# naturerobots/mesh_navigation

Measured on AMD Instinct MI355X. Metric: plans/sec (Dijkstra makePlan device path incl. computeVectorMap, 1M-vertex mesh), higher is better.
Workload: dtype f32

## Files before the change

### include/mnav.h

```cpp
#ifndef MNAV_H
#define MNAV_H

#include <stdint.h>

#ifdef __cplusplus
extern "C" {
#endif

#define MNAV_SUCCESS 0u
#define MNAV_CANCELED 51u
#define MNAV_INVALID_START 52u
#define MNAV_INVALID_GOAL 53u
#define MNAV_NO_PATH_FOUND 54u
#define MNAV_INTERNAL_ERROR 60u
#define MNAV_NONE 0xFFFFFFFFu

typedef struct mnav_ctx mnav_ctx;

typedef struct mnav_stats {
  uint32_t steps;
  uint32_t launches;
  uint32_t bands;
  uint32_t armed;
  float goal_dist;
// ... 73 lines not shown
                        const float* sensor_to_map, const float* down_axis, double robot_height, double max_obstacle_dist,
                        uint32_t* changed_out, uint32_t* n_changed, uint32_t* n_lethal);
int mnav_obstacle_stats(const mnav_ctx* ctx, uint32_t* rays_kept, uint32_t* hits, uint32_t* lethal_rays, float* ms_bvh_build,
                        float* ms_cast, float* ms_total);
int mnav_layer_height_diff(mnav_ctx* ctx, uint32_t layer, double radius, double threshold);
int mnav_layer_roughness(mnav_ctx* ctx, uint32_t layer, double radius, double threshold);
int mnav_layer_ridge(mnav_ctx* ctx, uint32_t layer, double radius, double threshold);
int mnav_neighbourhood_stats(const mnav_ctx* ctx, uint32_t* centres, uint64_t* visits, uint32_t* max_size,
                             uint32_t* spilled, float* ms);
int mnav_layer_border(mnav_ctx* ctx, uint32_t layer, double border_cost, double threshold, uint32_t* changed_out, uint32_t* n_changed,
                      uint32_t* n_lethal);
int mnav_layer_clearance(mnav_ctx* ctx, uint32_t layer, double robot_height, double height_inflation, uint32_t* changed_out,
                         uint32_t* n_changed, uint32_t* n_lethal);
int mnav_clearance_download(const mnav_ctx* ctx, float* clearance_out);
int mnav_clearance_stats(const mnav_ctx* ctx, uint32_t* cast, uint32_t* rays, uint32_t* hits, float* ms_bvh_build, float* ms_cast,
                         float* ms_total);

enum { MNAV_NODE_INPUT = 0, MNAV_NODE_INFLATION = 1, MNAV_NODE_COMBINE_MAX = 2, MNAV_NODE_COMBINE_AVG = 3 };
typedef struct {
  uint32_t layer;
  uint32_t kind;
  uint32_t n_inputs;
  uint32_t inputs[8];
  float    weights[8];
  double   inflation_radius, inscribed_radius, inscribed_value, lethal_value, cost_scaling_factor;
} mnav_map_node;
int mnav_map_configure(mnav_ctx* ctx, uint32_t n_nodes, const mnav_map_node* nodes, uint32_t default_layer, double edge_cost_factor,
                       const uint8_t* invalid);
int mnav_map_compute(mnav_ctx* ctx);
int mnav_map_layer_changed(mnav_ctx* ctx, uint32_t layer, uint32_t n, const uint32_t* vertex_ids, uint32_t* changed_out, uint32_t* n_changed);
int mnav_map_update_layer(mnav_ctx* ctx, uint32_t layer, uint32_t n, const uint32_t* vertex_ids, const float* costs, const uint8_t* lethal,
                          uint32_t* changed_out, uint32_t* n_changed);
int mnav_map_obstacle(mnav_ctx* ctx, uint32_t layer, uint32_t n_points, const void* points, uint32_t point_step, const float* sensor_to_map,
                      const float* down_axis, double robot_height, double max_obstacle_dist, uint32_t* changed_out, uint32_t* n_changed);
int mnav_map_stats(const mnav_ctx* ctx, uint32_t* waves, uint32_t* recombined, uint32_t* default_changed, uint32_t* edges_reweighted,
                   float* ms_total, float* ms_wave);

uint32_t mnav_replan_dijkstra_batch(mnav_ctx* ctx, uint32_t n, const uint32_t* targets, double goal_dist_offset, uint32_t* codes_out,
                                    float* dist_out, uint32_t* pred_out, uint32_t* path_out, uint32_t path_cap, uint32_t* path_len);
uint32_t mnav_replan_plans(const mnav_ctx* ctx);
int mnav_replan_stats(const mnav_ctx* ctx, uint32_t* reason, uint32_t* log_len, float* levels_out, uint64_t* kept, uint64_t* rewound,
                      uint32_t* tiles_woken, uint32_t* rounds, float* ms_level, float* ms_rewind, float* ms_rounds, float* ms_finalize);

uint32_t mnav_replan_dijkstra_each(mnav_ctx* ctx, uint32_t n, const uint32_t* targets, double goal_dist_offset, uint32_t* codes_out,
                                   float* dist_out, uint32_t* pred_out, uint32_t* path_out, uint32_t path_cap, uint32_t* path_len);
int mnav_replan_each_stats(const mnav_ctx* ctx, uint32_t* reason, uint32_t* whole_fresh, uint32_t* log_len, uint8_t* classes_out,
                           float* levels_out, uint32_t* counts, uint64_t* kept, uint64_t* rewound, uint32_t* tiles_woken, uint32_t* rounds,
                           int32_t* fresh_engine, float* ms);

int mnav_replan_warm_stats(const mnav_ctx* ctx, uint32_t* plans, uint32_t* kernel, uint32_t* iterations, uint64_t* pairs_woken, uint64_t* words,
                           float* ms, uint32_t* fallback, uint32_t* live);

int mnav_locate(mnav_ctx* ctx, uint32_t n, const float* pos, uint32_t* vertex_out, uint32_t* face_out, float* bary_out,
                float* dist_out);
int mnav_locate_stats(const mnav_ctx* ctx, uint32_t* built, float* ms_build, float* ms_query, uint64_t* candidates);
uint32_t mnav_plan_dijkstra_batch_at(mnav_ctx* ctx, uint32_t n, const float* goal_pos, const float* start_pos,
                                     double goal_dist_offset, double cost_limit, uint32_t* codes_out, uint32_t* seeds_out,
                                     uint32_t* targets_out, float* dist_out, uint32_t* pred_out, uint32_t* path_out,
                                     uint32_t path_cap, uint32_t* path_len);
uint32_t mnav_plan_cvp_batch_at(mnav_ctx* ctx, uint32_t n, const float* goal_pos, const float* start_pos,
                                double goal_dist_offset, double cost_limit, uint32_t* codes_out, uint32_t* seed_faces_out,
                                uint32_t* target_faces_out, float* dist_out, uint32_t* pred_out, float* vecmap_out);

typedef struct mnav_follow_config {
  double max_lin_velocity;
  double max_ang_velocity;
  double arrival_fading;
  double ang_vel_factor;
  double lin_vel_factor;
  double max_angle;
  double max_search_radius;
  double max_search_distance;
} mnav_follow_config;
#define MNAV_FOLLOW_CONFIG_DEFAULTS { 1.0, 0.5, 0.5, 1.0, 1.0, 20.0, 0.4, 0.4 }
enum { MNAV_FOLLOW_OK = 0, MNAV_FOLLOW_OUT_OF_MAP = 1, MNAV_FOLLOW_NO_FIELD = 2 };
int mnav_follow_batch(mnav_ctx* ctx, uint32_t n, const float* pos, const float* dir, const float* up, const uint32_t* face_in,
                      const uint32_t* slots, const uint32_t* seed_faces, const mnav_follow_config* config, int32_t* code_out,
                      uint32_t* face_out, float* bary_out, float* pos_out, float* mesh_dir_out, float* cost_out, double* cmd_out,
                      int32_t* how_out);
int mnav_follow_stats(const mnav_ctx* ctx, uint32_t* stayed, uint32_t* neighbour, uint32_t* global, uint32_t* lost,
                      uint32_t* no_field, uint32_t* built_index, float* ms_kernels, float* ms_total);

enum { MNAV_ROLLOUT_RUNNING = 0, MNAV_ROLLOUT_REACHED = 1, MNAV_ROLLOUT_OUT_OF_MAP = 2, MNAV_ROLLOUT_NO_FIELD = 3 };
typedef struct mnav_rollout_config {
  double   dt;
  double   dist_tolerance;
  double   angle_tolerance;
  uint32_t ticks;
  uint32_t trace_stride;
} mnav_rollout_config;
int mnav_follow_rollout(mnav_ctx* ctx, uint32_t n, const float* pos, const float* dir, const float* up, const uint32_t* face_in,
                        const uint32_t* slots, const uint32_t* seed_faces, const float* goal_pos, const float* goal_dir,
                        const mnav_follow_config* config, const mnav_rollout_config* rollout, int32_t* status_out,
                        uint32_t* ticks_out, float* pos_out, float* dir_out, uint32_t* face_out, double* travel_out,
                        double* cost_integral_out, float* min_goal_dist_out, float* trace_out);
int mnav_rollout_stats(const mnav_ctx* ctx, uint32_t* status_counts, uint64_t* robot_ticks, uint64_t* stayed, uint64_t* neighbour,
                       uint64_t* global, uint32_t* built_index, float* ms_kernels, float* ms_total);

#define MNAV_BEYOND_FIELD 70u
int mnav_fleet_paths(mnav_ctx* ctx, uint32_t n, const uint32_t* slots, const uint32_t* start_vertex, const float* start_pos,
                     uint32_t* code_out, uint32_t* vertex_out, float* potential_out, uint32_t* len_out, uint64_t* offset_out,
                     uint32_t* ids_out, uint64_t ids_cap, uint64_t* total_out);
int mnav_fleet_walks(mnav_ctx* ctx, uint32_t n, const uint32_t* slots, uint32_t n_plans, const float* seed_pos,
                     const uint32_t* seed_faces, const float* start_pos, const uint32_t* start_faces, double step_width,
                     int32_t inflation_layer, uint32_t walk_cap, int32_t* status_out, uint32_t* start_face_out, uint32_t* len_out,
                     uint64_t* offset_out, float* positions_out, uint32_t* faces_out, uint64_t entries_cap, uint64_t* total_out);
int mnav_upload_face_normals(mnav_ctx* ctx, uint32_t F, const float* face_normals);
int mnav_fleet_plans(mnav_ctx* ctx, uint32_t n, const uint32_t* slots, const uint32_t* start_vertex, const float* start_pos,
                     uint32_t n_plans, const float* goal_pos, uint32_t* code_out, uint32_t* vertex_out, float* potential_out,
                     uint32_t* len_out, uint64_t* offset_out, double* cost_out, double* poses_out, uint64_t poses_cap,
                     uint64_t* total_out);
int mnav_fleet_walk_plans(mnav_ctx* ctx, uint32_t n, const uint32_t* slots, uint32_t n_plans, const float* seed_pos,
                          const uint32_t* seed_faces, const double* goal_pose, const float* start_pos, const uint32_t* start_faces,
                          double step_width, int32_t inflation_layer, uint32_t walk_cap, int32_t* status_out,
                          uint32_t* start_face_out, uint32_t* len_out, uint64_t* offset_out, double* cost_out, double* poses_out,
                          uint64_t poses_cap, uint64_t* total_out);
int mnav_fleet_stats(const mnav_ctx* ctx, uint32_t* served, uint32_t* beyond_field, uint32_t* no_path, uint32_t* invalid,
                     uint64_t* entries, uint32_t* built_index, uint32_t* chunks, float* ms_kernels, float* ms_total);

int mnav_shard_setup(mnav_ctx* ctx, uint32_t rank, uint32_t world);
int mnav_shard_info(const mnav_ctx* ctx, uint32_t* t_lo, uint32_t* t_hi, uint32_t* ntiles, uint32_t* n_exchange);
int mnav_shard_setup_partition(mnav_ctx* ctx, uint32_t n_exchange, const uint32_t* exchange_vertex, const uint8_t* owned);
int mnav_shard_walk(mnav_ctx* ctx, uint32_t start_vertex, uint32_t seed_vertex, uint32_t cap, uint32_t* out_host);
uint64_t mnav_device_bytes(const mnav_ctx* ctx);

int mnav_shard_begin(mnav_ctx* ctx, uint32_t seed_vertex, uint32_t target_vertex, double goal_dist_offset, double cost_limit);
int mnav_shard_set_goal_tie(mnav_ctx* ctx, uint32_t tie_id);
int mnav_shard_rounds(mnav_ctx* ctx, uint32_t rounds, float* iface_buf_dev);
int mnav_shard_apply(mnav_ctx* ctx, const float* iface_buf_dev, float* local_min_out, float* target_dist_out);
int mnav_shard_finalize(mnav_ctx* ctx, float* dist_buf_dev, uint32_t* pred_buf_dev);
int mnav_shard_rounds_async(mnav_ctx* ctx, uint32_t rounds, float* iface_buf_dev, void* caller_stream);
int mnav_shard_apply_async(mnav_ctx* ctx, const float* iface_buf_dev, float* ctl_dev, void* caller_stream);

void mnav_cancel(mnav_ctx* ctx);

int mnav_get_stats(const mnav_ctx* ctx, mnav_stats* out);
int mnav_get_timing(const mnav_ctx* ctx, mnav_stats* out);
int mnav_set_band_width(mnav_ctx* ctx, float delta);
int mnav_set_dijkstra_engine(mnav_ctx* ctx, int engine);
int mnav_set_option(mnav_ctx* ctx, const char* name, double value);
double mnav_get_option(const mnav_ctx* ctx, const char* name);
int mnav_set_resident_outputs(mnav_ctx* ctx, int on);
int mnav_download_output(mnav_ctx* ctx, uint32_t slot, int what, void* host_out);
int mnav_vector_at(mnav_ctx* ctx, uint32_t slot, const uint32_t vs[3], const float bary[3], float out[3]);
int mnav_backtrack_cvp_batch(mnav_ctx* ctx, uint32_t n, const float* seed_pos, const uint32_t* seed_faces, const float* target_pos,
                             const uint32_t* target_faces, double step_width, int32_t inflation_layer, uint32_t cap,
                             float* positions_out, uint32_t* faces_out, uint32_t* n_out, int32_t* status_out);
int mnav_backtrack_cvp(mnav_ctx* ctx, const float seed_pos[3], uint32_t seed_face, const float target_pos[3], uint32_t target_face,
                       double step_width, int32_t inflation_layer, uint32_t cap, float* positions_out, uint32_t* faces_out,
                       uint32_t* n_out);
const void* mnav_device_output(const mnav_ctx* ctx, uint32_t slot, int what);
uint64_t mnav_algorithmic_bytes(const mnav_ctx* ctx);
int mnav_last_engine(const mnav_ctx* ctx);

#ifdef __cplusplus
}
#endif
#endif
```

### mesh_navigation_amd/capi.py

```python
from __future__ import annotations

import ctypes as C
import os
import sys
import time
import weakref
from dataclasses import dataclass

import numpy as np

from . import build as _build

NONE = 0xFFFFFFFF
SUCCESS, CANCELED, INVALID_START, INVALID_GOAL, NO_PATH_FOUND, INTERNAL_ERROR = 0, 51, 52, 53, 54, 60
BEYOND_FIELD = 70
WALK_NO_FACE = -3

SYMBOLS = [
    "mnav_create", "mnav_destroy", "mnav_last_error", "mnav_set_face_circulation", "mnav_upload_mesh", "mnav_upload_costs",
    "mnav_compute_edge_weights", "mnav_combine_costs", "mnav_plan_dijkstra", "mnav_plan_cvp", "mnav_plan_dijkstra_batch", "mnav_plan_cvp_batch",
    "mnav_cancel", "mnav_get_stats", "mnav_get_timing", "mnav_set_band_width", "mnav_set_dijkstra_engine", "mnav_device_output",
    "mnav_algorithmic_bytes", "mnav_shard_setup", "mnav_shard_setup_partition", "mnav_shard_walk", "mnav_device_bytes", "mnav_shard_info", "mnav_shard_begin", "mnav_shard_rounds", "mnav_shard_apply", "mnav_shard_rounds_async", "mnav_shard_apply_async",
    "mnav_shard_finalize", "mnav_update_costs", "mnav_update_edge_weights", "mnav_download_costs", "mnav_set_resident_outputs", "mnav_download_output",
    "mnav_vector_at", "mnav_backtrack_cvp", "mnav_backtrack_cvp_batch", "mnav_layer_upload", "mnav_layer_steepness", "mnav_layer_inflation", "mnav_layer_download",
    "mnav_combine_layers", "mnav_layer_stats", "mnav_layer_download_vectors", "mnav_combine_layers_update",
    "mnav_layer_obstacle", "mnav_obstacle_stats",
    "mnav_layer_height_diff", "mnav_layer_roughness", "mnav_layer_ridge", "mnav_neighbourhood_stats",
    "mnav_layer_border", "mnav_layer_clearance", "mnav_clearance_download", "mnav_clearance_stats",
    "mnav_locate", "mnav_locate_stats", "mnav_plan_dijkstra_batch_at", "mnav_plan_cvp_batch_at",
    "mnav_follow_batch", "mnav_follow_stats", "mnav_follow_rollout", "mnav_rollout_stats",
    "mnav_map_configure", "mnav_map_compute", "mnav_map_layer_changed", "mnav_map_update_layer", "mnav_map_obstacle", "mnav_map_stats",
    "mnav_replan_dijkstra_batch", "mnav_replan_plans", "mnav_replan_stats", "mnav_replan_dijkstra_each", "mnav_replan_each_stats",
    "mnav_replan_warm_stats",
    "mnav_fleet_paths", "mnav_fleet_walks", "mnav_fleet_stats",
    "mnav_upload_face_normals", "mnav_fleet_plans", "mnav_fleet_walk_plans",
    "mnav_set_option", "mnav_get_option", "mnav_shard_set_goal_tie", "mnav_last_engine",
]


class _PathRows:

    def __init__(self, buf, lens, cap):
        self._buf, self._lens, self._cap = buf, lens, cap

    def __len__(self):
        return self._lens.shape[0]

    def __getitem__(self, k):
        if isinstance(k, slice):
            return [self[i] for i in range(*k.indices(len(self)))]
        if k < 0:
            k += len(self)
        return self._buf[k, : min(int(self._lens[k]), self._cap)].copy()

    def __iter__(self):
        return (self[i] for i in range(len(self)))


class Stats(C.Structure):
    _fields_ = [("steps", C.c_uint32), ("launches", C.c_uint32), ("bands", C.c_uint32), ("armed", C.c_uint32),
                ("goal_dist", C.c_float), ("n_plans", C.c_uint32), ("evals", C.c_uint64), ("settled", C.c_uint64),
                ("ms_init", C.c_float), ("ms_propagation", C.c_float), ("ms_vector_map", C.c_float),
                ("ms_path", C.c_float), ("ms_download", C.c_float), ("ms_total", C.c_float), ("ms_step_kernels", C.c_float),
                ("band_shrinks", C.c_uint32), ("band_cuts", C.c_uint32)]

    def as_dict(self) -> dict:
        return {k: getattr(self, k) for k, _ in self._fields_}


class FollowConfig(C.Structure):
    _fields_ = [("max_lin_velocity", C.c_double), ("max_ang_velocity", C.c_double), ("arrival_fading", C.c_double),
                ("ang_vel_factor", C.c_double), ("lin_vel_factor", C.c_double), ("max_angle", C.c_double),
                ("max_search_radius", C.c_double), ("max_search_distance", C.c_double)]
    DEFAULTS = dict(max_lin_velocity=1.0, max_ang_velocity=0.5, arrival_fading=0.5, ang_vel_factor=1.0, lin_vel_factor=1.0,
                    max_angle=20.0, max_search_radius=0.4, max_search_distance=0.4)

    def __init__(self, **kw):
        super().__init__(**{**self.DEFAULTS, **kw})


FOLLOW_OK, FOLLOW_OUT_OF_MAP, FOLLOW_NO_FIELD = 0, 1, 2


class RolloutConfig(C.Structure):
    _fields_ = [("dt", C.c_double), ("dist_tolerance", C.c_double), ("angle_tolerance", C.c_double), ("ticks", C.c_uint32),
                ("trace_stride", C.c_uint32)]
    DEFAULTS = dict(dt=0.1, dist_tolerance=0.2, angle_tolerance=0.8, ticks=1, trace_stride=0)

    def __init__(self, **kw):
        super().__init__(**{**self.DEFAULTS, **kw})


ROLLOUT_RUNNING, ROLLOUT_REACHED, ROLLOUT_OUT_OF_MAP, ROLLOUT_NO_FIELD = 0, 1, 2, 3


class MapNode(C.Structure):
    _fields_ = [("layer", C.c_uint32), ("kind", C.c_uint32), ("n_inputs", C.c_uint32), ("inputs", C.c_uint32 * 8),
                ("weights", C.c_float * 8), ("inflation_radius", C.c_double), ("inscribed_radius", C.c_double),
                ("inscribed_value", C.c_double), ("lethal_value", C.c_double), ("cost_scaling_factor", C.c_double)]


NODE_KINDS = {"input": 0, "inflation": 1, "max": 2, "avg": 3}


@dataclass
class FollowOut:
    code: np.ndarray | None
    face: np.ndarray | None
    bary: np.ndarray | None
    pos: np.ndarray | None
    mesh_dir: np.ndarray | None
    cost: np.ndarray | None
    cmd: np.ndarray | None
    how: np.ndarray | None


@dataclass
class RolloutOut:
    status: np.ndarray | None
    ticks: np.ndarray | None
    pos: np.ndarray | None
    dir: np.ndarray | None
    face: np.ndarray | None
    travel: np.ndarray | None
    cost_integral: np.ndarray | None
    min_goal_dist: np.ndarray | None
    trace: np.ndarray | None
    cancelled: bool = False


_lib = None


def load(path: str | None = None):
    global _lib
    if _lib is not None and path is None:
        return _lib
    p = path or os.environ.get("MNAV_LIB") or _build.LIB
    if path is None and not os.path.exists(p):
        _build.build_lib()
    if not os.path.exists(p):
        raise RuntimeError(f"HIP library {p} is missing -- run `python -m mesh_navigation_amd.build`")
    L = C.CDLL(p)
    vp, u32, f64 = C.c_void_p, C.c_uint32, C.c_double
    L.mnav_create.restype = vp
    L.mnav_create.argtypes = [C.c_int]
    L.mnav_destroy.argtypes = [vp]
    L.mnav_last_error.restype = C.c_char_p
    L.mnav_last_error.argtypes = [vp]
    L.mnav_set_face_circulation.restype = C.c_int
    L.mnav_set_face_circulation.argtypes = [vp, u32, u32, vp, vp]
    L.mnav_upload_mesh.restype = C.c_int
    L.mnav_upload_mesh.argtypes = [vp, u32, u32, u32, vp, vp, vp, vp]
    L.mnav_upload_costs.restype = C.c_int
    L.mnav_upload_costs.argtypes = [vp, vp, vp, vp]
    L.mnav_compute_edge_weights.restype = C.c_int
    L.mnav_compute_edge_weights.argtypes = [vp, vp, vp, f64, vp, vp]
    L.mnav_combine_costs.restype = C.c_int
    L.mnav_combine_costs.argtypes = [vp, C.c_int, u32, vp, vp, vp, f64, vp, vp, vp]
    L.mnav_plan_dijkstra.restype = u32
    L.mnav_plan_dijkstra.argtypes = [vp, u32, u32, f64, f64, vp, vp, vp, u32, C.POINTER(u32), vp]
    L.mnav_plan_cvp.restype = u32
    L.mnav_plan_cvp.argtypes = [vp, vp, u32, u32, f64, f64, vp, vp, vp, vp, vp]
    L.mnav_plan_dijkstra_batch.restype = u32
    L.mnav_plan_dijkstra_batch.argtypes = [vp, u32, vp, vp, f64, f64, vp, vp, vp, vp, u32, vp]
    L.mnav_plan_cvp_batch.restype = u32
    L.mnav_plan_cvp_batch.argtypes = [vp, u32, vp, vp, vp, f64, f64, vp, vp, vp, vp]
    L.mnav_locate.restype = C.c_int
    L.mnav_locate.argtypes = [vp, u32, vp, vp, vp, vp, vp]
    L.mnav_locate_stats.restype = C.c_int
    L.mnav_locate_stats.argtypes = [vp, C.POINTER(u32), C.POINTER(C.c_float), C.POINTER(C.c_float), C.POINTER(C.c_uint64)]
    L.mnav_plan_dijkstra_batch_at.restype = u32
    L.mnav_plan_dijkstra_batch_at.argtypes = [vp, u32, vp, vp, f64, f64, vp, vp, vp, vp, vp, vp, u32, vp]
    L.mnav_plan_cvp_batch_at.restype = u32
    L.mnav_plan_cvp_batch_at.argtypes = [vp, u32, vp, vp, f64, f64, vp, vp, vp, vp, vp, vp]
    L.mnav_follow_batch.restype = C.c_int
    L.mnav_follow_batch.argtypes = [vp, u32, vp, vp, vp, vp, vp, vp, C.POINTER(FollowConfig), vp, vp, vp, vp, vp, vp, vp, vp]
    L.mnav_follow_stats.restype = C.c_int
    L.mnav_follow_stats.argtypes = [vp] + [C.POINTER(u32)] * 6 + [C.POINTER(C.c_float)] * 2
    L.mnav_follow_rollout.restype = C.c_int
    L.mnav_follow_rollout.argtypes = [vp, u32] + [vp] * 8 + [C.POINTER(FollowConfig), C.POINTER(RolloutConfig)] + [vp] * 9
    L.mnav_rollout_stats.restype = C.c_int
    L.mnav_rollout_stats.argtypes = [vp, C.POINTER(u32 * 4)] + [C.POINTER(C.c_uint64)] * 4 + [C.POINTER(u32)] + [C.POINTER(C.c_float)] * 2
    L.mnav_map_configure.restype = C.c_int
    L.mnav_map_configure.argtypes = [vp, u32, C.POINTER(MapNode), u32, f64, vp]
    L.mnav_map_compute.restype = C.c_int
    L.mnav_map_compute.argtypes = [vp]
    L.mnav_map_layer_changed.restype = C.c_int
    L.mnav_map_layer_changed.argtypes = [vp, u32, u32, vp, vp, C.POINTER(u32)]
    L.mnav_map_update_layer.restype = C.c_int
    L.mnav_map_update_layer.argtypes = [vp, u32, u32, vp, vp, vp, vp, C.POINTER(u32)]
    L.mnav_map_obstacle.restype = C.c_int
    L.mnav_map_obstacle.argtypes = [vp, u32, u32, vp, u32, vp, vp, f64, f64, vp, C.POINTER(u32)]
    L.mnav_map_stats.restype = C.c_int
    L.mnav_map_stats.argtypes = [vp] + [C.POINTER(u32)] * 4 + [C.POINTER(C.c_float)] * 2
    L.mnav_replan_dijkstra_batch.restype = u32
    L.mnav_replan_dijkstra_batch.argtypes = [vp, u32, vp, f64, vp, vp, vp, vp, u32, vp]
    L.mnav_replan_dijkstra_each.restype = u32
    L.mnav_replan_dijkstra_each.argtypes = [vp, u32, vp, f64, vp, vp, vp, vp, u32, vp]
    L.mnav_replan_each_stats.restype = C.c_int
    L.mnav_replan_each_stats.argtypes = ([vp] + [C.POINTER(u32)] * 3 + [vp, vp, vp] + [C.POINTER(C.c_uint64)] * 2 + [C.POINTER(u32)] * 2
                                         + [C.POINTER(C.c_int32), vp])
    L.mnav_replan_warm_stats.restype = C.c_int
    L.mnav_replan_warm_stats.argtypes = [vp] + [C.POINTER(u32)] * 3 + [C.POINTER(C.c_uint64)] * 2 + [vp] + [C.POINTER(u32)] * 2
    L.mnav_replan_plans.restype = u32
    L.mnav_replan_plans.argtypes = [vp]
    L.mnav_replan_stats.restype = C.c_int
    L.mnav_replan_stats.argtypes = [vp, C.POINTER(u32), C.POINTER(u32), vp] + [C.POINTER(C.c_uint64)] * 2 + [C.POINTER(u32)] * 2 + [C.POINTER(C.c_float)] * 4
    L.mnav_cancel.argtypes = [vp]
    L.mnav_get_stats.restype = C.c_int
    L.mnav_get_stats.argtypes = [vp, C.POINTER(Stats)]
    L.mnav_get_timing.restype = C.c_int
    L.mnav_get_timing.argtypes = [vp, C.POINTER(Stats)]
    L.mnav_set_band_width.restype = C.c_int
    L.mnav_set_band_width.argtypes = [vp, C.c_float]
    L.mnav_set_dijkstra_engine.restype = C.c_int
    L.mnav_set_dijkstra_engine.argtypes = [vp, C.c_int]
    L.mnav_shard_set_goal_tie.restype = C.c_int
    L.mnav_shard_set_goal_tie.argtypes = [vp, u32]
    L.mnav_set_option.restype = C.c_int
    L.mnav_set_option.argtypes = [vp, C.c_char_p, C.c_double]
    L.mnav_get_option.restype = C.c_double
    L.mnav_get_option.argtypes = [vp, C.c_char_p]
    L.mnav_device_output.restype = vp
    L.mnav_device_output.argtypes = [vp, u32, C.c_int]
    L.mnav_set_resident_outputs.restype = C.c_int
    L.mnav_set_resident_outputs.argtypes = [vp, C.c_int]
    L.mnav_download_output.restype = C.c_int
    L.mnav_download_output.argtypes = [vp, u32, C.c_int, vp]
    L.mnav_backtrack_cvp_batch.restype = C.c_int
    L.mnav_backtrack_cvp_batch.argtypes = [vp, u32, vp, vp, vp, vp, C.c_double, C.c_int32, u32, vp, vp, vp, vp]
    L.mnav_backtrack_cvp.restype = C.c_int
    L.mnav_backtrack_cvp.argtypes = [vp, vp, u32, vp, u32, C.c_double, C.c_int32, u32, vp, vp, vp]
    L.mnav_vector_at.restype = C.c_int
    L.mnav_vector_at.argtypes = [vp, u32, vp, vp, vp]
    L.mnav_update_costs.restype = C.c_int
    L.mnav_update_costs.argtypes = [vp, u32, vp, vp]
    L.mnav_update_edge_weights.restype = C.c_int
    L.mnav_update_edge_weights.argtypes = [vp, u32, vp, vp]
    L.mnav_download_costs.restype = C.c_int
    L.mnav_download_costs.argtypes = [vp, vp, vp]
    L.mnav_layer_upload.restype = C.c_int
    L.mnav_layer_upload.argtypes = [vp, u32, vp, vp]
    L.mnav_layer_steepness.restype = C.c_int
    L.mnav_layer_steepness.argtypes = [vp, u32, f64]
    L.mnav_layer_inflation.restype = C.c_int
    L.mnav_layer_inflation.argtypes = [vp, u32, u32, f64, f64, f64, f64, f64, vp]
    L.mnav_layer_download.restype = C.c_int
    L.mnav_layer_download.argtypes = [vp, u32, vp, vp, vp]
    L.mnav_combine_layers_update.restype = C.c_int
    L.mnav_combine_layers_update.argtypes = [vp, C.c_int, u32, vp, vp, u32, vp]
    L.mnav_layer_download_vectors.restype = C.c_int
    L.mnav_layer_download_vectors.argtypes = [vp, u32, vp, vp]
    L.mnav_combine_layers.restype = C.c_int
    L.mnav_combine_layers.argtypes = [vp, C.c_int, u32, vp, vp, f64, vp]
    L.mnav_layer_stats.restype = C.c_int
    L.mnav_layer_stats.argtypes = [vp, C.POINTER(u32), C.POINTER(u32), C.POINTER(C.c_uint64), C.POINTER(C.c_float), C.POINTER(u32), C.POINTER(C.c_float)]
    L.mnav_layer_obstacle.restype = C.c_int
    L.mnav_layer_obstacle.argtypes = [vp, u32, u32, vp, u32, vp, vp, f64, f64, vp, C.POINTER(u32), C.POINTER(u32)]
    L.mnav_obstacle_stats.restype = C.c_int
    L.mnav_obstacle_stats.argtypes = [vp, C.POINTER(u32), C.POINTER(u32), C.POINTER(u32), C.POINTER(C.c_float), C.POINTER(C.c_float), C.POINTER(C.c_float)]
    for name in ("mnav_layer_height_diff", "mnav_layer_roughness", "mnav_layer_ridge"):
        getattr(L, name).restype = C.c_int
        getattr(L, name).argtypes = [vp, u32, f64, f64]
    L.mnav_neighbourhood_stats.restype = C.c_int
    L.mnav_neighbourhood_stats.argtypes = [vp, C.POINTER(u32), C.POINTER(C.c_uint64), C.POINTER(u32), C.POINTER(u32), C.POINTER(C.c_float)]
    for name in ("mnav_layer_border", "mnav_layer_clearance"):
        getattr(L, name).restype = C.c_int
        getattr(L, name).argtypes = [vp, u32, f64, f64, vp, C.POINTER(u32), C.POINTER(u32)]
    L.mnav_clearance_download.restype = C.c_int
    L.mnav_clearance_download.argtypes = [vp, vp]
    L.mnav_clearance_stats.restype = C.c_int
    L.mnav_clearance_stats.argtypes = [vp, C.POINTER(u32), C.POINTER(u32), C.POINTER(u32), C.POINTER(C.c_float), C.POINTER(C.c_float), C.POINTER(C.c_float)]
    L.mnav_shard_setup.restype = C.c_int
    L.mnav_shard_setup.argtypes = [vp, u32, u32]
    L.mnav_shard_setup_partition.restype = C.c_int
    L.mnav_shard_setup_partition.argtypes = [vp, u32, C.POINTER(u32), C.POINTER(C.c_uint8)]
    L.mnav_shard_walk.restype = C.c_int
    L.mnav_shard_walk.argtypes = [vp, u32, u32, u32, C.POINTER(u32)]
    L.mnav_device_bytes.restype = C.c_uint64
    L.mnav_device_bytes.argtypes = [vp]
    L.mnav_shard_info.restype = C.c_int
    L.mnav_shard_info.argtypes = [vp, C.POINTER(u32), C.POINTER(u32), C.POINTER(u32), C.POINTER(u32)]
    L.mnav_shard_begin.restype = C.c_int
    L.mnav_shard_begin.argtypes = [vp, u32, u32, f64, f64]
    L.mnav_shard_rounds.restype = C.c_int
    L.mnav_shard_rounds.argtypes = [vp, u32, vp]
    L.mnav_shard_rounds_async.restype = C.c_int
    L.mnav_shard_rounds_async.argtypes = [vp, u32, vp, vp]
    L.mnav_shard_apply_async.restype = C.c_int
    L.mnav_shard_apply_async.argtypes = [vp, vp, vp, vp]
    L.mnav_shard_apply.restype = C.c_int
    L.mnav_shard_apply.argtypes = [vp, vp, C.POINTER(C.c_float), C.POINTER(C.c_float)]
    L.mnav_shard_finalize.restype = C.c_int
    L.mnav_shard_finalize.argtypes = [vp, vp, vp]
    L.mnav_algorithmic_bytes.restype = C.c_uint64
    L.mnav_algorithmic_bytes.argtypes = [vp]
    L.mnav_last_engine.restype = C.c_int
    L.mnav_last_engine.argtypes = [vp]
    L.mnav_fleet_paths.restype = C.c_int
    L.mnav_fleet_paths.argtypes = [vp, u32] + [vp] * 9 + [C.c_uint64, vp]
    L.mnav_fleet_walks.restype = C.c_int
    L.mnav_fleet_walks.argtypes = [vp, u32, vp, u32, vp, vp, vp, vp, f64, C.c_int32, u32] + [vp] * 6 + [C.c_uint64, vp]
    L.mnav_upload_face_normals.restype = C.c_int
    L.mnav_upload_face_normals.argtypes = [vp, u32, vp]
    L.mnav_fleet_plans.restype = C.c_int
    L.mnav_fleet_plans.argtypes = [vp, u32, vp, vp, vp, u32] + [vp] * 8 + [C.c_uint64, vp]
    L.mnav_fleet_walk_plans.restype = C.c_int
    L.mnav_fleet_walk_plans.argtypes = [vp, u32, vp, u32, vp, vp, vp, vp, vp, f64, C.c_int32, u32] + [vp] * 6 + [C.c_uint64, vp]
    L.mnav_fleet_stats.restype = C.c_int
    L.mnav_fleet_stats.argtypes = [vp] + [C.POINTER(u32)] * 4 + [C.POINTER(C.c_uint64)] + [C.POINTER(u32)] * 2 + [C.POINTER(C.c_float)] * 2
    if path is None:
        _lib = L
    return L


def _p(a):
    return None if a is None else a.ctypes.data_as(C.c_void_p)


def _f32(a):
    return np.ascontiguousarray(a, dtype=np.float32)


def _u32(a):
    return np.ascontiguousarray(a, dtype=np.uint32)


def quat_to_matrix(q_wxyz, translation) -> np.ndarray:
    f = np.float32
    q = np.asarray(q_wxyz, f).reshape(4)
    nrm = np.sqrt(((q[0] * q[0] + q[1] * q[1]) + q[2] * q[2]) + q[3] * q[3], dtype=f)
    w, x, y, z = (q / nrm).astype(f)
    tx, ty, tz = f(2) * x, f(2) * y, f(2) * z
    twx, twy, twz = tx * w, ty * w, tz * w
    txx, txy, txz = tx * x, ty * x, tz * x
    tyy, tyz, tzz = ty * y, tz * y, tz * z
    one = f(1)
    R = np.array([[one - (tyy + tzz), txy - twz, txz + twy],
                  [txy + twz, one - (txx + tzz), tyz - twx],
                  [txz - twy, tyz + twx, one - (txx + tyy)]], f)
    return np.ascontiguousarray(np.concatenate([R, np.asarray(translation, f).reshape(3, 1)], axis=1), f)


@dataclass
class DijkstraOut:
    code: int
    dist: np.ndarray | None
    pred: np.ndarray | None
    path: np.ndarray
    vecmap: np.ndarray | None
    stats: dict


@dataclass
class CvpOut:
    code: int
    dist: np.ndarray | None
    pred: np.ndarray | None
    direction: np.ndarray | None
    cutface: np.ndarray | None
    vecmap: np.ndarray | None
    stats: dict


def _engine_name(e: int) -> str:
    return {0: "k_tile_round (tile rounds)", 1: "k_step (band steps)", 5: "k_tb_solve_q (tile-batch engine, quarters of a wave, distances in LDS)",
            21: "k_tbv_solve (tile-batch engine, one wave per tile, distances in VGPRs)", 6: "k_plan_async (asynchronous tile engine)"}.get(e, "none")


def _warm_name(kernel: int) -> str:
    return "k_tb_warm + %s (tile-batch engine started from the rewound fields)" % ("k_tbv_solve" if kernel == 1 else "k_tb_solve_q")


class MnavContext:

    def __init__(self, device: int = 0):
        self._L = load()
        self._h = self._L.mnav_create(int(device))
        if not self._h:
            raise RuntimeError("mnav_create failed: no usable MI355X/HIP device (there is no CPU fallback)")
        self.V = self.F = self.E = 0

    def close(self):
        if getattr(self, "_h", None):
            self._L.mnav_destroy(self._h)
            self._h = None

    def __del__(self):
        try:
            self.close()
        except Exception:
            pass

    def __enter__(self):
        return self

    def __exit__(self, *a):
        self.close()

    def _err(self) -> str:
        return (self._L.mnav_last_error(self._h) or b"").decode()

    def upload_mesh(self, xyz, faces, edges, vertex_normals=None, face_circulation=None):
        xyz, faces, edges = _f32(xyz), _u32(faces), _u32(edges)
        vn = None if vertex_normals is None else _f32(vertex_normals)
        self.V, self.F, self.E = xyz.shape[0], faces.shape[0], edges.shape[0]
        if face_circulation is not None:
            ptr, vf = _u32(face_circulation[0]), _u32(face_circulation[1])
            self._L.mnav_set_face_circulation(self._h, self.V, self.F, _p(ptr), _p(vf))
        else:
            self._L.mnav_set_face_circulation(self._h, self.V, self.F, None, None)
        rc = self._L.mnav_upload_mesh(self._h, self.V, self.F, self.E, _p(xyz), _p(faces), _p(edges), _p(vn))
        if rc != 0:
            raise RuntimeError(f"mnav_upload_mesh failed ({rc}): {self._err()}")

    def upload_costs(self, vertex_costs, edge_weights, invalid=None):
        vc, w = _f32(vertex_costs), _f32(edge_weights)
        inv = None if invalid is None else np.ascontiguousarray(invalid, dtype=np.uint8)
        rc = self._L.mnav_upload_costs(self._h, _p(vc), _p(w), _p(inv))
        if rc != 0:
            raise RuntimeError(f"mnav_upload_costs failed ({rc}): {self._err()}")

    def compute_edge_weights(self, vertex_costs, edge_distances, edge_cost_factor: float, invalid=None) -> np.ndarray:
        vc, ed = _f32(vertex_costs), _f32(edge_distances)
        inv = None if invalid is None else np.ascontiguousarray(invalid, dtype=np.uint8)
        out = np.empty(self.E, dtype=np.float32)
        rc = self._L.mnav_compute_edge_weights(self._h, _p(vc), _p(ed), float(edge_cost_factor), _p(inv), _p(out))
        if rc != 0:
            raise RuntimeError(f"mnav_compute_edge_weights failed ({rc}): {self._err()}")
        return out

    def combine_costs(self, layers, weights, edge_distances, edge_cost_factor: float, mode: str = "avg", invalid=None):
        arrs = [_f32(a) for a in layers]
        ptrs = (C.c_void_p * max(len(arrs), 1))(*[a.ctypes.data for a in arrs])
        w = _f32(weights if weights is not None else np.ones(len(arrs), np.float32))
        ed = _f32(edge_distances)
        inv = None if invalid is None else np.ascontiguousarray(invalid, dtype=np.uint8)
        vc = np.empty(self.V, dtype=np.float32)
        ew = np.empty(self.E, dtype=np.float32)
        rc = self._L.mnav_combine_costs(self._h, 0 if mode == "max" else 1, len(arrs), C.cast(ptrs, C.c_void_p), _p(w), _p(ed),
                                        float(edge_cost_factor), _p(inv), _p(vc), _p(ew))
        if rc != 0:
            raise RuntimeError(f"mnav_combine_costs failed ({rc}): {self._err()}")
        return vc, ew

    def set_band_width(self, delta: float):
        self._L.mnav_set_band_width(self._h, float(delta))

    def set_dijkstra_engine(self, engine: str):
        if self._L.mnav_set_dijkstra_engine(self._h, {"tiled": 0, "band": 1, "auto": 3, "tile_batch": 5, "async": 6}[engine]) != 0:
            raise ValueError(f"engine {engine!r} refused")
# ... 179 lines not shown
        if self._L.mnav_layer_download_vectors(self._h, int(layer), _p(vec), _p(has)) != 0:
            raise RuntimeError(f"mnav_layer_download_vectors failed: {self._err()}")
        return vec, has

    def combine_layers(self, layers, weights=None, mode: str = "avg", edge_cost_factor: float = 1.0, invalid=None):
        ls = np.ascontiguousarray(layers, np.uint32)
        w = np.ascontiguousarray(weights if weights is not None else [1.0] * len(ls), np.float32)
        inv = None if invalid is None else np.ascontiguousarray(invalid, np.uint8)
        if self._L.mnav_combine_layers(self._h, 0 if mode == "max" else 1, len(ls), _p(ls), _p(w), float(edge_cost_factor),
                                       None if inv is None else _p(inv)) != 0:
            raise RuntimeError(f"mnav_combine_layers failed: {self._err()}")

    def combine_layers_update(self, layers, ids, weights=None, mode: str = "avg"):
        ls = np.ascontiguousarray(layers, np.uint32)
        w = np.ascontiguousarray(weights if weights is not None else [1.0] * len(ls), np.float32)
        ii = np.ascontiguousarray(ids, np.uint32)
        if self._L.mnav_combine_layers_update(self._h, 0 if mode == "max" else 1, len(ls), _p(ls), _p(w), ii.shape[0], _p(ii)) != 0:
            raise RuntimeError(f"mnav_combine_layers_update failed: {self._err()}")

    def map_configure(self, nodes, default_layer: int, edge_cost_factor: float = 0.0, invalid=None):
        arr = (MapNode * max(len(nodes), 1))()
        for a, n in zip(arr, nodes):
            ins = list(n.get("inputs", ()))
            if len(ins) > 8:
                raise ValueError("a node takes at most 8 inputs")
            ws = list(n.get("weights", [1.0] * len(ins)))
            a.layer, a.kind, a.n_inputs = int(n["layer"]), NODE_KINDS[n["kind"]], len(ins)
            for k, i in enumerate(ins):
                a.inputs[k] = int(i)
            for k, w in enumerate(ws[:8]):
                a.weights[k] = float(w)
            a.inflation_radius = float(n.get("inflation_radius", 0.4))
            a.inscribed_radius = float(n.get("inscribed_radius", 0.25))
            a.inscribed_value = float(n.get("inscribed_value", 0.99))
            a.lethal_value = float(n.get("lethal_value", 1.0))
            a.cost_scaling_factor = float(n.get("cost_scaling_factor", 1.0))
        inv = None if invalid is None else np.ascontiguousarray(invalid, np.uint8)
        if self._L.mnav_map_configure(self._h, len(nodes), arr, int(default_layer), float(edge_cost_factor),
                                      None if inv is None else _p(inv)) != 0:
            raise RuntimeError(f"mnav_map_configure failed: {self._err()}")

    def map_compute(self):
        if self._L.mnav_map_compute(self._h) != 0:
            raise RuntimeError(f"mnav_map_compute failed: {self._err()}")

    def _map_call(self, name: str, layer: int, *args) -> dict:
        changed = np.empty(max(self.V, 1), np.uint32)
        nc = C.c_uint32()
        if getattr(self._L, name)(self._h, int(layer), *args, _p(changed), C.byref(nc)) != 0:
            raise RuntimeError(f"{name} failed: {self._err()}")
        return dict(changed=changed[:nc.value].copy(), stats=self.map_stats())

    def map_layer_changed(self, layer: int, ids) -> dict:
        ii = np.ascontiguousarray(ids, np.uint32).reshape(-1)
        return self._map_call("mnav_map_layer_changed", layer, ii.shape[0], _p(ii))

    def map_update_layer(self, layer: int, ids, costs, lethal=None) -> dict:
        ii = np.ascontiguousarray(ids, np.uint32).reshape(-1)
        cc = np.ascontiguousarray(costs, np.float32).reshape(-1)
        le = None if lethal is None else np.ascontiguousarray(lethal, np.uint8).reshape(-1)
        if cc.shape[0] != ii.shape[0] or (le is not None and le.shape[0] != ii.shape[0]):
            raise ValueError("ids, costs and lethal must have one length")
        return self._map_call("mnav_map_update_layer", layer, ii.shape[0], _p(ii), _p(cc), None if le is None else _p(le))

    def map_obstacle(self, layer: int, points, sensor_to_map=None, rotation_wxyz=None, translation=None,
                     down_axis=(0.0, 0.0, -1.0), robot_height: float = np.inf, max_obstacle_dist: float = np.inf) -> dict:
        args = self._obstacle_args(points, sensor_to_map, rotation_wxyz, translation, down_axis, robot_height, max_obstacle_dist)
        return self._map_call("mnav_map_obstacle", layer, *args[1:])

    def map_stats(self) -> dict:
        w, r, d, e, mt, mw = C.c_uint32(), C.c_uint32(), C.c_uint32(), C.c_uint32(), C.c_float(), C.c_float()
        self._L.mnav_map_stats(self._h, C.byref(w), C.byref(r), C.byref(d), C.byref(e), C.byref(mt), C.byref(mw))
        return dict(waves=w.value, recombined=r.value, default_changed=d.value, edges_reweighted=e.value, ms_total=mt.value, ms_wave=mw.value)

    def shard_setup(self, rank: int, world: int) -> int:
        n = self._L.mnav_shard_setup(self._h, int(rank), int(world))
        if n < 0:
            raise RuntimeError(f"mnav_shard_setup failed: {self._err()}")
        return n

    def shard_setup_partition(self, exchange_vertex: np.ndarray, owned: np.ndarray) -> int:
        ex = np.ascontiguousarray(exchange_vertex, np.uint32)
        ow = np.ascontiguousarray(owned, np.uint8)
        if ow.shape[0] != self.V:
            raise ValueError("owned: one byte per local vertex")
        n = self._L.mnav_shard_setup_partition(self._h, ex.shape[0], ex.ctypes.data_as(C.POINTER(C.c_uint32)), ow.ctypes.data_as(C.POINTER(C.c_uint8)))
        if n < 0:
            raise RuntimeError(f"mnav_shard_setup_partition failed: {self._err()}")
        return n

    def shard_walk(self, start: int, seed: int, cap: int = 4096) -> np.ndarray:
        out = np.zeros(cap + 3, np.uint32)
        if self._L.mnav_shard_walk(self._h, int(start), int(seed), int(cap), out.ctypes.data_as(C.POINTER(C.c_uint32))) != 0:
            raise RuntimeError(f"mnav_shard_walk failed: {self._err()}")
        return out

    def device_bytes(self) -> int:
        return int(self._L.mnav_device_bytes(self._h))

    def shard_info(self) -> dict:
        a, b, c, d = C.c_uint32(), C.c_uint32(), C.c_uint32(), C.c_uint32()
        if self._L.mnav_shard_info(self._h, C.byref(a), C.byref(b), C.byref(c), C.byref(d)) != 0:
            raise RuntimeError("mnav_shard_setup has not been called")
        return dict(t_lo=a.value, t_hi=b.value, ntiles=c.value, n_exchange=d.value)

    def shard_set_goal_tie(self, tie_id: int):
        self._L.mnav_shard_set_goal_tie(self._h, int(tie_id))

    def shard_begin(self, seed: int, target: int, goal_dist_offset: float = 0.3, cost_limit: float = 1.0):
        if self._L.mnav_shard_begin(self._h, int(seed), int(target), float(goal_dist_offset), float(cost_limit)) != 0:
            raise RuntimeError(f"mnav_shard_begin failed: {self._err()}")

    def shard_rounds(self, rounds: int, buf_ptr: int) -> int:
        rc = self._L.mnav_shard_rounds(self._h, int(rounds), C.c_void_p(buf_ptr))
        if rc < 0:
            raise RuntimeError(f"mnav_shard_rounds failed: {self._err()}")
        return rc

    def shard_apply(self, buf_ptr: int):
        lm, td = C.c_float(), C.c_float()
        if self._L.mnav_shard_apply(self._h, C.c_void_p(buf_ptr), C.byref(lm), C.byref(td)) != 0:
            raise RuntimeError(f"mnav_shard_apply failed: {self._err()}")
        return lm.value, td.value

    def shard_rounds_async(self, rounds: int, buf_ptr: int, stream: int):
        if self._L.mnav_shard_rounds_async(self._h, int(rounds), C.c_void_p(buf_ptr), C.c_void_p(stream)) != 0:
            raise RuntimeError(f"mnav_shard_rounds_async failed: {self._err()}")

    def shard_apply_async(self, buf_ptr: int, ctl_ptr: int, stream: int):
        if self._L.mnav_shard_apply_async(self._h, C.c_void_p(buf_ptr), C.c_void_p(ctl_ptr), C.c_void_p(stream)) != 0:
            raise RuntimeError(f"mnav_shard_apply_async failed: {self._err()}")

    def shard_finalize(self, dist_ptr: int, pred_ptr: int):
        rc = self._L.mnav_shard_finalize(self._h, C.c_void_p(dist_ptr), C.c_void_p(pred_ptr))
        if rc != 0:
            raise RuntimeError(f"mnav_shard_finalize failed ({rc}): {self._err()}")

    def stats(self) -> dict:
        s = Stats()
        self._L.mnav_get_stats(self._h, C.byref(s))
        d = s.as_dict()
        d["algorithmic_bytes"] = int(self._L.mnav_algorithmic_bytes(self._h))
        return d

    def last_engine(self) -> str:
        e = int(self._L.mnav_last_engine(self._h))
        if e >= 256:
            ran = (["k_tile_round (tile rounds)"] if e & 128 else []) + ([_warm_name(1 if e & 1024 else 0)] if e & 512 else [])
            ran += [_engine_name(e & 127)] if (e & 127) != 127 else []
            return " + ".join(ran) if ran else "none (every plan kept)"
        if e in (5, 21) and self.replan_warm_stats()["live"]:
            return _warm_name(1 if e == 21 else 0)
        return _engine_name(e)

    def timing(self) -> dict:
        s = Stats()
        self._L.mnav_get_timing(self._h, C.byref(s))
        return s.as_dict()

    def cancel(self):
        self._L.mnav_cancel(self._h)

    def device_output(self, slot: int, what: int) -> int:
        return int(self._L.mnav_device_output(self._h, slot, what) or 0)

    def plan_dijkstra(self, seed_vertex: int, target_vertex: int, goal_dist_offset: float = 0.3,
                      cost_limit: float = 1.0, want_fields: bool = True, want_vecmap: bool = False) -> DijkstraOut:
        V = self.V
        dist = np.empty(V, np.float32) if want_fields else None
        pred = np.empty(V, np.uint32) if want_fields else None
        vm = np.empty((V, 3), np.float32) if want_vecmap else None
        path = np.empty(max(V, 1), np.uint32)
        n = C.c_uint32(0)
        code = self._L.mnav_plan_dijkstra(self._h, int(seed_vertex) & 0xFFFFFFFF, int(target_vertex) & 0xFFFFFFFF,
                                          float(goal_dist_offset), float(cost_limit), _p(dist), _p(pred), _p(path),
                                          path.shape[0], C.byref(n), _p(vm))
        if code == INTERNAL_ERROR:
            raise RuntimeError(f"mnav_plan_dijkstra internal error: {self._err()}")
        return DijkstraOut(code, dist, pred, path[: n.value].copy(), vm, self.stats())

    def _lease_paths(self, n: int, cap: int):
        key = (n, max(cap, 1))
        if getattr(self, "_path_buf_key", None) != key:
            self._path_pool, self._path_buf_key = [], key
        paths = None
        for entry in self._path_pool:
            entry[1] = [r for r in entry[1] if r() is not None]
            if not entry[1]:
                paths = entry[0]
                lease = entry[1]
                break
        if paths is None:
            paths = np.empty(key, np.uint32)
            lease = []
            if len(self._path_pool) < 3:
                self._path_pool.append([paths, lease])
        return paths, lease

    def plan_dijkstra_batch(self, seeds, targets, goal_dist_offset: float = 0.3, cost_limit: float = 1.0,
                            want_fields: bool = False, path_cap: int | None = None, want_stats: bool = True):
        seeds, targets = _u32(seeds), _u32(targets)
        n = seeds.shape[0]
        V = self.V
        cap = int(path_cap if path_cap is not None else V)
        codes = np.empty(n, np.uint32)
        dist = np.empty((n, V), np.float32) if want_fields else None
        pred = np.empty((n, V), np.uint32) if want_fields else None
        paths, lease = self._lease_paths(n, cap)
        lens = np.zeros(n, np.uint32)
        rc = self._L.mnav_plan_dijkstra_batch(self._h, n, _p(seeds), _p(targets), float(goal_dist_offset),
                                              float(cost_limit), _p(codes), _p(dist), _p(pred), _p(paths), cap, _p(lens))
        if rc == INTERNAL_ERROR:
            raise RuntimeError(f"mnav_plan_dijkstra_batch internal error: {self._err()}")
        rows = _PathRows(paths, lens, cap)
        lease.append(weakref.ref(rows))
        return dict(rc=rc, codes=codes, dist=dist, pred=pred, paths=rows, path_len=lens,
                    stats=self.stats() if want_stats else self.timing())

    def replan_dijkstra(self, targets=None, goal_dist_offset: float = 0.3, want_dist: bool = False, want_pred: bool = False,
                        path_cap: int | None = None, want_stats: bool = True):
        n = int(self._L.mnav_replan_plans(self._h)) if targets is None else int(_u32(targets).shape[0])
        tg = None if targets is None else _u32(targets)
        V = self.V
        cap = int(path_cap if path_cap is not None else V)
        codes = np.empty(n, np.uint32)
        dist = np.empty((n, V), np.float32) if want_dist else None
        pred = np.empty((n, V), np.uint32) if want_pred else None
        paths, lease = self._lease_paths(n, cap)
        lens = np.zeros(n, np.uint32)
        rc = self._L.mnav_replan_dijkstra_batch(self._h, n, _p(tg), float(goal_dist_offset), _p(codes), _p(dist), _p(pred), _p(paths), cap, _p(lens))
        if rc == INTERNAL_ERROR:
            raise RuntimeError(f"mnav_replan_dijkstra_batch internal error: {self._err()}")
        rows = _PathRows(paths, lens, cap)
        lease.append(weakref.ref(rows))
        return dict(rc=rc, codes=codes, dist=dist, pred=pred, paths=rows, path_len=lens, stats=self.stats() if want_stats else self.timing(),
                    replan=self.replan_stats(n) if want_stats else None, warm=self.replan_warm_stats() if want_stats else None)

    def replan_dijkstra_each(self, targets=None, goal_dist_offset: float = 0.3, want_dist: bool = False, want_pred: bool = False,
                             path_cap: int | None = None, want_stats: bool = True):
        n = int(self._L.mnav_replan_plans(self._h)) if targets is None else int(_u32(targets).shape[0])
        tg = None if targets is None else _u32(targets)
        V = self.V
        cap = int(path_cap if path_cap is not None else V)
        codes = np.empty(n, np.uint32)
        dist = np.empty((n, V), np.float32) if want_dist else None
        pred = np.empty((n, V), np.uint32) if want_pred else None
        paths, lease = self._lease_paths(n, cap)
        lens = np.zeros(n, np.uint32)
        rc = self._L.mnav_replan_dijkstra_each(self._h, n, _p(tg), float(goal_dist_offset), _p(codes), _p(dist), _p(pred), _p(paths), cap, _p(lens))
        if rc == INTERNAL_ERROR:
            raise RuntimeError(f"mnav_replan_dijkstra_each internal error: {self._err()}")
        rows = _PathRows(paths, lens, cap)
        lease.append(weakref.ref(rows))
        return dict(rc=rc, codes=codes, dist=dist, pred=pred, paths=rows, path_len=lens, stats=self.stats() if want_stats else self.timing(),
                    replan=self.replan_stats(n) if want_stats else None, each=self.replan_each_stats(n) if want_stats else None,
                    warm=self.replan_warm_stats() if want_stats else None)

    def replan_warm_stats(self) -> dict:
        pl, kn, it, fb, lv = (C.c_uint32() for _ in range(5))
        wk, wd = C.c_uint64(), C.c_uint64()
        ms = np.zeros(3, np.float32)
        self._L.mnav_replan_warm_stats(self._h, C.byref(pl), C.byref(kn), C.byref(it), C.byref(wk), C.byref(wd), _p(ms), C.byref(fb), C.byref(lv))
        why = {0: None, 1: "more than 65535 repaired plans", 2: "the tile-batch engine could not be allocated"}.get(fb.value, str(fb.value))
        return dict(plans=pl.value, kernel=("k_tbv_solve" if kn.value == 1 else "k_tb_solve_q") if pl.value else None, iterations=it.value,
                    pairs_woken=wk.value, words=wd.value, ms_warm=float(ms[0]), ms_engine=float(ms[1]), ms_finalize=float(ms[2]),
                    fallback=fb.value, fallback_reason=why, live=bool(lv.value))

    def replan_each_stats(self, n: int = 0) -> dict:
        r, wf, ll, tw, rd = (C.c_uint32() for _ in range(5))
        k, w = C.c_uint64(), C.c_uint64()
        fe = C.c_int32()
        counts = np.zeros(3, np.uint32)
        ms = np.zeros(5, np.float32)
        self._L.mnav_replan_each_stats(self._h, C.byref(r), C.byref(wf), C.byref(ll), None, None, _p(counts), C.byref(k), C.byref(w), C.byref(tw),
                                       C.byref(rd), C.byref(fe), _p(ms))
        cls = lv = None
        if n and int(counts.sum()) == n:
            cls, lv = np.zeros(n, np.uint8), np.zeros(n, np.float32)
            self._L.mnav_replan_each_stats(self._h, None, None, None, _p(cls), _p(lv), *([None] * 7))
        return dict(reason=r.value, whole_fresh=bool(wf.value), log_len=ll.value, classes=cls, levels=lv, kept_plans=int(counts[0]),
                    repaired_plans=int(counts[1]), fresh_plans=int(counts[2]), kept=k.value, rewound=w.value, tiles_woken=tw.value,
                    rounds=rd.value, fresh_engine=_engine_name(fe.value) if fe.value >= 0 else None, ms_classify=float(ms[0]),
                    ms_rewind=float(ms[1]), ms_rounds=float(ms[2]), ms_finalize=float(ms[3]), ms_fresh=float(ms[4]))

    def replan_stats(self, n: int = 0) -> dict:
        r, ll, tw, rd = (C.c_uint32() for _ in range(4))
        k, w = C.c_uint64(), C.c_uint64()
        ms = [C.c_float() for _ in range(4)]
        self._L.mnav_replan_stats(self._h, C.byref(r), C.byref(ll), None, C.byref(k), C.byref(w), C.byref(tw), C.byref(rd), *[C.byref(x) for x in ms])
        lv = None
        if r.value == 0 and n:
            lv = np.zeros(n, np.float32)
            self._L.mnav_replan_stats(self._h, None, None, _p(lv), *([None] * 8))
        return dict(reason=r.value, log_len=ll.value, levels=lv, kept=k.value, rewound=w.value, tiles_woken=tw.value, rounds=rd.value,
                    ms_level=ms[0].value, ms_rewind=ms[1].value, ms_rounds=ms[2].value, ms_finalize=ms[3].value)

    def fleet_paths(self, slots, start_vertex=None, start_pos=None, ids_cap: int | None = None) -> dict:
        sl = _u32(slots).reshape(-1)
        n = int(sl.shape[0])
        sv = None if start_vertex is None else _u32(start_vertex).reshape(-1)
        sp = None if start_pos is None else _f32(start_pos).reshape(-1, 3)
        if (sv is not None and sv.shape[0] != n) or (sv is None and sp is not None and sp.shape[0] != n):
            raise ValueError("fleet_paths: the per-robot arrays differ in length")
        codes, vtx, lens = (np.zeros(n, np.uint32) for _ in range(3))
        pot = np.zeros(n, np.float32)
        off = np.zeros(n + 1, np.uint64)
# ... 283 lines not shown
```

### mesh_navigation_amd/csrc/mnav.hip

```cpp
#include <hip/hip_runtime.h>

#include <algorithm>
#include <array>
#include <atomic>
#include <chrono>
#include <cmath>
#include <cstdio>
#include <cstdlib>
#include <cstring>
#include <functional>
#include <map>
#include <string>
#include <vector>
#include <unordered_map>
#include <unistd.h>

#include "../../include/mnav.h"
#include "mnav_buf.h"
#include "mnav_build.h"
#include "mnav_eval.h"
#include "mnav_options.h"

using namespace mnav;

// ... 1760 lines not shown
    if (slot >= ctx->last_n) { ctx->err = "output not resident"; return -1; }
    if (hipSetDevice(ctx->device) != hipSuccess) return -1;
    DevBuf<float> tmp;
    HIPCHK(tmp.alloc(4 * (size_t)(ctx->V ? ctx->V : 1)));
    const uint32_t g = std::min<uint32_t>((ctx->V + kBlock - 1) / kBlock + 1, 4096);
    if (ctx->last_engine == 5 && ctx->lazy_paths && !ctx->tb_args_valid) { ctx->err = "output not resident"; return -1; }
    if (ctx->last_engine == 5 && ctx->lazy_paths) hipLaunchKernelGGL(k_tb_popped, dim3(g), dim3(kBlock), 0, ctx->stream, ctx->tb_args, slot, ctx->V, tmp);
    else hipLaunchKernelGGL(k_popped, dim3(g), dim3(kBlock), 0, ctx->stream, ctx->slots[slot].dist, ctx->last_target[slot], ctx->last_offset, ctx->V, tmp);
    const hipError_t e1 = hipMemcpyAsync(host_out, tmp, 4 * (size_t)ctx->V, hipMemcpyDeviceToHost, ctx->stream);
    const hipError_t e2 = hipStreamSynchronize(ctx->stream);
    tmp.reset();
    if (e1 != hipSuccess || e2 != hipSuccess) { ctx->err = "popped potential: copy failed"; return -1; }
    return 0;
  }
  const void* src = mnav_device_output(ctx, slot, what);
  if (!src) { ctx->err = "output not resident"; return -1; }
  if (hipSetDevice(ctx->device) != hipSuccess) return -1;
  const size_t bytes = (what == 4 ? 12 : 4) * (size_t)ctx->V;
  HIPCHK(hipMemcpyAsync(host_out, src, bytes, hipMemcpyDeviceToHost, ctx->stream));
  HIPCHK(hipStreamSynchronize(ctx->stream));
  return 0;
}

int mnav_vector_at(mnav_ctx* ctx, uint32_t slot, const uint32_t vs[3], const float bary[3], float out[3])
{
  if (!ctx || !vs || !bary || !out) return -1;
  for (int k = 0; k < 3; ++k) if (vs[k] >= ctx->V) { ctx->err = "vertex id out of range"; return -1; }
  float v[3][3];
  if (ctx->last_planner == kPlannerDijkstra && ctx->last_engine == 5 && ctx->lazy_paths && ctx->tb_args_valid) {
    uint32_t p = slot;
    if (p < ctx->caller_slot.size()) p = ctx->caller_slot[p];
    if (p >= ctx->last_n) { ctx->err = "output not resident"; return -1; }
    if (hipSetDevice(ctx->device) != hipSuccess) return -1;
    if (!ctx->d_vec3) HIPCHK(ctx->d_vec3.alloc(64));
    hipLaunchKernelGGL(k_tb_vector3, dim3(3), dim3(kWave), 0, ctx->stream, ctx->tb_args, ctx->d_row_ptr, ctx->d_nbr, ctx->d_xyz, p,
                       make_uint3(vs[0], vs[1], vs[2]), ctx->d_vec3);
    HIPCHK(hipGetLastError());
    HIPCHK(hipMemcpyAsync(&v[0][0], ctx->d_vec3, 36, hipMemcpyDeviceToHost, ctx->stream));
    HIPCHK(hipStreamSynchronize(ctx->stream));
  } else {
    const float* vm = static_cast<const float*>(mnav_device_output(ctx, slot, 4));
    if (!vm) { ctx->err = "vector map not resident"; return -1; }
    if (hipSetDevice(ctx->device) != hipSuccess) return -1;
    for (int k = 0; k < 3; ++k) HIPCHK(hipMemcpyAsync(v[k], vm + 3 * (size_t)vs[k], 12, hipMemcpyDeviceToHost, ctx->stream));
    HIPCHK(hipStreamSynchronize(ctx->stream));
  }
  float acc[3] = { 0.f, 0.f, 0.f };
  bool any = false;
  for (int k = 0; k < 3; ++k) {
    const bool has = !(v[k][0] == 0.f && v[k][1] == 0.f && v[k][2] == 0.f);
    if (!has) continue;
    any = true;
    for (int c = 0; c < 3; ++c) acc[c] += v[k][c] * bary[k];
  }
  if (!any || !(std::isfinite(acc[0]) && std::isfinite(acc[1]) && std::isfinite(acc[2]))) return 0;
  out[0] = acc[0]; out[1] = acc[1]; out[2] = acc[2];
  return 1;
}

int mnav_backtrack_cvp_batch(mnav_ctx* ctx, uint32_t n, const float* seed_pos, const uint32_t* seed_faces, const float* target_pos,
                             const uint32_t* target_faces, double step_width, int32_t inflation_layer, uint32_t cap, float* positions_out,
                             uint32_t* faces_out, uint32_t* n_out, int32_t* status_out)
{
  if (!ctx) return -1;
  ctx->err.clear();
  if (!n) return 0;
  if (!seed_pos || !seed_faces || !target_pos || !target_faces || !positions_out || !faces_out || !n_out || !status_out) { ctx->err = "null argument"; return -1; }
  if (cap < 2 || (uint64_t)cap * n > (1ull << 28)) { ctx->err = "path capacity out of range"; return -1; }
  if (!(step_width > 0.0)) { ctx->err = "step_width must be positive"; return -1; }
  if (ctx->last_planner != kPlannerCvp) { ctx->err = "back-tracking: the last call was not a CVP plan"; return -1; }
  if (hipSetDevice(ctx->device) != hipSuccess) { ctx->err = "hipSetDevice failed"; return -1; }
  if (n != ctx->caller_slot.size()) { ctx->err = "back-tracking: n differs from the last mnav_plan_cvp(_batch) call"; return -1; }
  std::vector<WalkJob> jobs(n);
  for (uint32_t i = 0; i < n; ++i) {
    const float* vm = static_cast<const float*>(mnav_device_output(ctx, i, 4));
    jobs[i].vecmap = nullptr;
    if (ctx->caller_slot[i] == kNone) continue;
    if (!vm) { ctx->err = "vector map not resident (mnav_set_resident_outputs, or pass vecmap_out to the plan call)"; return -1; }
    if (seed_faces[i] >= ctx->F || target_faces[i] >= ctx->F) { ctx->err = "face id out of range"; return -1; }
    jobs[i].vecmap = vm; jobs[i].seed_face = seed_faces[i]; jobs[i].target_face = target_faces[i];
    for (int k = 0; k < 3; ++k) { jobs[i].seed[k] = seed_pos[3 * (size_t)i + k]; jobs[i].target[k] = target_pos[3 * (size_t)i + k]; }
  }
  WalkInflation L{};
  if (inflation_layer >= 0) {
    if ((size_t)inflation_layer >= ctx->layers.size() || !ctx->layers[inflation_layer].ready || !ctx->layers[inflation_layer].dist || !ctx->layers[inflation_layer].have_vec) {
      ctx->err = "back-tracking: not a resident inflation layer with a vector field"; return -1;
    }
    const mnav_ctx::Layer& Ly = ctx->layers[inflation_layer];
    L.distances = Ly.dist; L.vectors = Ly.vec; L.has_vector = Ly.vstate;
    L.inflation_radius = Ly.inflation_radius; L.inscribed_radius = Ly.inscribed_radius; L.inscribed_value = Ly.inscribed_value; L.lethal_value = Ly.lethal_value;
    L.repulsive_field = 1;
  }
  if (upload_walk_mesh(ctx)) return -1;
  const size_t need = (size_t)cap * n;
  if (need > ctx->walk_cap) {
    ctx->d_walk_pos.reset(); ctx->d_walk_face.reset(); ctx->walk_cap = 0;
    HIPCHK(ctx->d_walk_pos.alloc(12 * need)); HIPCHK(ctx->d_walk_face.alloc(4 * need));
    ctx->walk_cap = need;
  }
  if (n > ctx->walk_jobs_cap) {
    ctx->d_walk_jobs.reset(); ctx->d_walk_ctl.reset(); ctx->walk_jobs_cap = 0;
    HIPCHK(ctx->d_walk_jobs.alloc(sizeof(WalkJob) * (size_t)n)); HIPCHK(ctx->d_walk_ctl.alloc(8 * (size_t)n));
    ctx->walk_jobs_cap = n;
  }
  HIPCHK(hipMemcpyAsync(ctx->d_walk_jobs, jobs.data(), sizeof(WalkJob) * (size_t)n, hipMemcpyHostToDevice, ctx->stream));
  WalkMesh M{ ctx->d_xyz, ctx->d_faces, ctx->d_vf_ptr, ctx->d_vf, ctx->V, ctx->F };
  hipLaunchKernelGGL(k_backtrack, dim3(n), dim3(64), 0, ctx->stream, M, L, ctx->d_walk_jobs, step_width, cap, ctx->d_walk_pos, ctx->d_walk_face, ctx->d_walk_ctl);
  HIPCHK(hipGetLastError());
  std::vector<int32_t> ctl(2 * (size_t)n);
  HIPCHK(hipMemcpyAsync(ctl.data(), ctx->d_walk_ctl, 8 * (size_t)n, hipMemcpyDeviceToHost, ctx->stream));
  HIPCHK(hipStreamSynchronize(ctx->stream));
  for (uint32_t i = 0; i < n; ++i) {
    const uint32_t m = (uint32_t)ctl[2 * (size_t)i + 1];
    if (m) {
      HIPCHK(hipMemcpyAsync(positions_out + 3 * (size_t)cap * i, ctx->d_walk_pos + 3 * (size_t)cap * i, 12 * (size_t)m, hipMemcpyDeviceToHost, ctx->stream));
      HIPCHK(hipMemcpyAsync(faces_out + (size_t)cap * i, ctx->d_walk_face + (size_t)cap * i, 4 * (size_t)m, hipMemcpyDeviceToHost, ctx->stream));
    }
  }
  HIPCHK(hipStreamSynchronize(ctx->stream));
  for (uint32_t i = 0; i < n; ++i) {
    const uint32_t m = (uint32_t)ctl[2 * (size_t)i + 1];
    float* pp = positions_out + 3 * (size_t)cap * i; uint32_t* pf = faces_out + (size_t)cap * i;
    for (uint32_t a = 0, b = m ? m - 1 : 0; a < b; ++a, --b) {
      for (int k = 0; k < 3; ++k) std::swap(pp[3 * (size_t)a + k], pp[3 * (size_t)b + k]);
      std::swap(pf[a], pf[b]);
    }
    n_out[i] = m; status_out[i] = ctl[2 * (size_t)i];
  }
  return 0;
}

int mnav_backtrack_cvp(mnav_ctx* ctx, const float seed_pos[3], uint32_t seed_face, const float target_pos[3], uint32_t target_face, double step_width,
                       int32_t inflation_layer, uint32_t cap, float* positions_out, uint32_t* faces_out, uint32_t* n_out)
{
  int32_t status = 0;
  const int rc = mnav_backtrack_cvp_batch(ctx, 1, seed_pos, &seed_face, target_pos, &target_face, step_width, inflation_layer, cap, positions_out, faces_out, n_out, &status);
  return rc < 0 ? rc : status;
}

uint64_t mnav_algorithmic_bytes(const mnav_ctx* ctx)
{
  if (!ctx) return 0;
  settle_stats(const_cast<mnav_ctx*>(ctx));
  return ctx->algo_bytes;
}

int mnav_last_engine(const mnav_ctx* ctx)
{
  if (!ctx || ctx->last_planner != kPlannerDijkstra || ctx->last_n == 0) return -1;
  if (ctx->rp.each_engines) return ctx->rp.each_engines;
  return ctx->last_engine + ((ctx->last_engine == 5 && ctx->tb.kernel == 1) ? 16 : 0);
}

#ifdef MNAV_TILE_TIMING
int mnav_debug_tile_timing(unsigned long long* out, unsigned int cap)
{
  unsigned int n = 0;
  (void)hipMemcpyFromSymbol(&n, HIP_SYMBOL(g_tile_timing_n), sizeof(n));
  if (n > 4096) n = 4096;
  if (n > cap) n = cap;
  (void)hipMemcpyFromSymbol(out, HIP_SYMBOL(g_tile_timing), sizeof(unsigned long long) * 8 * n);
  unsigned int z = 0;
  (void)hipMemcpyToSymbol(HIP_SYMBOL(g_tile_timing_n), &z, sizeof(z));
  return (int)n;
}
#endif

}

#ifdef MNAV_WIDE_TIMING
extern "C" int mnav_debug_wide_timing(unsigned long long* out)
{
  if (hipMemcpyFromSymbol(out, HIP_SYMBOL(g_wide_timing), sizeof(unsigned long long) * 12) != hipSuccess) return -1;
  unsigned long long z[12] = { 0, 0, 0, 0, 0, 0, 0, 0, 0, 0, 0, 0 };
  return hipMemcpyToSymbol(HIP_SYMBOL(g_wide_timing), z, sizeof(z)) == hipSuccess ? 0 : -1;
}
#endif
```

### mesh_navigation_amd/csrc/mnav_options.h

```cpp
#pragma once

#define MNAV_OPTION_LIST(X)                                                                                                              \
  X(verbose)                                                              \
  X(trace)                                                                                       \
  X(no_graph)             \
  X(debug_chunk)                                                                            \
  X(dijkstra_engine)                                 \
  X(blocks_per_plan)                                                                                 \
  X(tile_blocks)                                                                                    \
  X(cvp_wide)                                        \
  X(wide_waves)                                                                                      \
  X(cvp_groups)                          \
  X(max_steps) X(max_wall_s)                                                                                                             \
  X(cvp_verify)                                                                     \
  X(key_walk_max) X(descend_walk_max)                                                               \
  X(tile_size)                                                                                   \
  X(lazy_paths)                                                                                      \
  X(tile_band) X(rounds_band_mult)                                                                                                       \
  X(tb_tile)                                                       \
  X(tb_no_prefill) X(tb_band_mult) X(tb_waves_per_cu)                                                                                    \
  X(tb_kernel)            \
  X(async_wg_per_cu) X(async_wg_per_plan) X(async_max_s)                                                                                 \
  X(async_band_mult)                              \
  X(async_max_batch)                                           \
  X(async_ring_cap)             \
  X(nbhd_lds_cap)         \
  X(replan_log_cap)                                          \
  X(replan_fresh_below)   \
  X(replan_each_fresh_share)  \
  X(replan_repair_engine)  \
  X(replan_warm_min_plans)  \
  X(fleet_scratch_mb)

struct Options {
#define X(name) double name = NAN;
  MNAV_OPTION_LIST(X)
#undef X
  struct Desc { const char* name; double Options::*field; };
  static const Desc* table(size_t* n)
  {
    static const Desc t[] = {
#define X(name) { #name, &Options::name },
      MNAV_OPTION_LIST(X)
#undef X
    };
    *n = sizeof(t) / sizeof(t[0]);
    return t;
  }
  double* find(const char* name)
  {
    size_t n; const Desc* t = table(&n);
    for (size_t i = 0; i < n; ++i) if (!strcmp(t[i].name, name)) return &(this->*t[i].field);
    return nullptr;
  }
  void from_environment()
  {
    size_t n; const Desc* t = table(&n);
    for (size_t i = 0; i < n; ++i) {
      std::string var = "MNAV_";
      for (const char* c = t[i].name; *c; ++c) var += (char)toupper((unsigned char)*c);
      const char* e = getenv(var.c_str());
      if (!e || !*e) continue;
      double v = atof(e);
      if (!strcmp(t[i].name, "dijkstra_engine")) {
        v = !strcmp(e, "tiled") ? 0 : !strcmp(e, "band") ? 1 : !strcmp(e, "tile_batch") ? 5 : !strcmp(e, "async") ? 6
          : (e[0] >= '0' && e[0] <= '9') ? atof(e) : 3;
      }
      this->*t[i].field = v;
    }
  }
};
static inline bool opt_set(double v) { return v == v; }
static inline uint32_t opt_u32(double v, uint32_t dflt) { return v == v ? (uint32_t)(v < 0.0 ? 0.0 : v) : dflt; }
static inline bool opt_on(double v) { return v == v && v != 0.0; }
```

### mesh_navigation_amd/csrc/mnav_tb.h

```cpp
#pragma once

#include "mnav_tb_build.h"

namespace {

namespace tb {

#define MNAV_CONST __attribute__((address_space(4)))
typedef uint32_t u32x16 __attribute__((ext_vector_type(16)));
typedef const MNAV_CONST u32x16* cblk8_t;
typedef __attribute__((address_space(3))) uint32_t* lds_u32_t;
enum { kTwSoff = 0, kTwSl = 1, kTwNv = 2, kTwNh = 3, kTwSweepOff = 4, kTwSweepChunks = 5, kTwPreOff = 6, kTwPreChunks = 7,
       kTwPostOff = 8, kTwPostChunks = 9, kTwExpOff = 10, kTwExpN = 11 };
static_assert(offsetof(TbTile, exp_n) == 4 * kTwExpN && offsetof(TbTile, sweep_off) == 4 * kTwSweepOff, "TbTile layout");

struct Ctl {
  uint32_t n_cand[2];
  uint32_t n_items, next_item;
  uint32_t err;
  uint32_t iters;
  unsigned long long acts;
  unsigned long long sweeps;
  unsigned long long items;
  unsigned long long wakes;
// ... 587 lines not shown
      }
      TB_STAMP(6);
    }
  }
#ifdef MNAV_TB_TIMING
  if (lane == 0) for (int k = 0; k < 8; ++k) if (tt[k]) atomicAdd(&g_tb_timing[k], tt[k]);
#endif
  my_wakes = wave_sum(my_wakes); my_acts = wave_sum(my_acts);
  if (__any(my_first != 0u) && lane == 0) A.ctl->n_cand[par ^ 1] = 1u;
  if (lane == 0 && my_items && blockIdx.x < A.wstat_slots) {
    unsigned long long* const ws = A.wstat + 4u * blockIdx.x;
    ws[0] += (unsigned long long)my_items; ws[1] += (unsigned long long)my_acts; ws[2] += (unsigned long long)my_sweeps; ws[3] += (unsigned long long)my_wakes;
  }
}

__global__ __launch_bounds__(kWave) void k_tb_path(tb::Args A, const uint32_t* __restrict__ row_ptr, const Nbr* __restrict__ nbr, uint32_t V,
                                                   PlanResult* __restrict__ res, PathRows rows, uint32_t* __restrict__ mismatch)
{
  const uint32_t p = blockIdx.x;
  if (rows.skip(p)) return;
  const int lane = threadIdx.x;
  PlanResult& R = res[p];
  const uint32_t seed = A.seed[p], target = A.target[p];
  const float dt = A.D[tb::slot_addr(A.vaddr[target], A.NP, p)];
  const GoalCut gcut = goal_cut(dt, A.offset, target);
  const float goal_dist = gcut.goal;
  uint32_t code = kSuccess, n = 0, bad = 0;
  if (A.ctl->err || A.ctl->n_cand[0]) code = kInternalError;
  else if (!(dt < inf_f())) code = kNoPathFound;
  else {
    uint32_t* path = rows.row(p);
    const uint32_t cap = rows.capacity(p);
    uint32_t v = target;
    float dv = dt;
    while (v != seed && n <= V) {
      float best_s = inf_f(), best_du = inf_f();
      uint32_t best_u = v;
      const uint32_t beg = row_ptr[v], end = row_ptr[v + 1];
      for (uint32_t i = beg + lane; i < end; i += kWave) {
        const Nbr nb = nbr[i];
        const float du = A.D[tb::slot_addr(A.vaddr[nb.u], A.NP, p)];
        if (!expanded_source(gcut, du, nb.u)) continue;
        const float sm = du + nb.w;
        if (sm < best_s || (sm == best_s && sm < inf_f() && (du < best_du || (du == best_du && nb.u < best_u)))) { best_s = sm; best_du = du; best_u = nb.u; }
      }
#pragma unroll
      for (int o = 1; o < kWave; o <<= 1) {
        const float os = __shfl_xor(best_s, o), odu = __shfl_xor(best_du, o);
        const uint32_t ou = __shfl_xor(best_u, o);
        if (os < best_s || (os == best_s && os < inf_f() && (odu < best_du || (odu == best_du && ou < best_u)))) { best_s = os; best_du = odu; best_u = ou; }
      }
      if (f2u(best_s) != f2u(dv) || best_u == v) { bad = 1; break; }
      v = best_u; dv = best_du;
      if (lane == 0 && n < cap) path[n] = v;
      ++n;
    }
    if (bad || v != seed) code = kInternalError;
    else if (n > cap) code = kPathOverflow;
  }
  if (lane == 0) {
    R.code = code; R.path_len = (code == kSuccess || code == kPathOverflow) ? n : 0;
    R.steps = A.ctl->iters; R.bands = 0; R.armed = (dt < inf_f()) ? 1u : 0u; R.overflow = A.ctl->err;
    R.goal_dist = goal_dist; R.evals = 0; R.shrinks = 0;
    if (bad) atomicAdd(mismatch, 1u);
  }
}

__global__ __launch_bounds__(kWave) void k_tb_vector3(tb::Args A, const uint32_t* __restrict__ row_ptr, const Nbr* __restrict__ nbr,
                                                      const float* __restrict__ xyz, uint32_t p, uint3 vs, float* __restrict__ out)
{
  const int lane = threadIdx.x;
  const uint32_t v = blockIdx.x == 0 ? vs.x : blockIdx.x == 1 ? vs.y : vs.z;
  const float dt = A.D[tb::slot_addr(A.vaddr[A.target[p]], A.NP, p)];
  const GoalCut gcut = goal_cut(dt, A.offset, A.target[p]);
  float best_s = inf_f(), best_du = inf_f();
  uint32_t best_u = v;
  if (v != A.seed[p]) {
    const uint32_t beg = row_ptr[v], end = row_ptr[v + 1];
    for (uint32_t i = beg + lane; i < end; i += kWave) {
      const Nbr nb = nbr[i];
      const float du = A.D[tb::slot_addr(A.vaddr[nb.u], A.NP, p)];
      if (!expanded_source(gcut, du, nb.u)) continue;
      const float sm = du + nb.w;
      if (sm < best_s || (sm == best_s && sm < inf_f() && (du < best_du || (du == best_du && nb.u < best_u)))) { best_s = sm; best_du = du; best_u = nb.u; }
    }
#pragma unroll
    for (int o = 1; o < kWave; o <<= 1) {
      const float os = __shfl_xor(best_s, o), odu = __shfl_xor(best_du, o);
      const uint32_t ou = __shfl_xor(best_u, o);
      if (os < best_s || (os == best_s && os < inf_f() && (odu < best_du || (odu == best_du && ou < best_u)))) { best_s = os; best_du = odu; best_u = ou; }
    }
    if (!(best_s < inf_f())) best_u = v;
  }
  if (lane == 0) {
    float x = 0.f, y = 0.f, z = 0.f;
    if (best_u != v) {
      x = xyz[3 * (size_t)best_u] - xyz[3 * (size_t)v];
      y = xyz[3 * (size_t)best_u + 1] - xyz[3 * (size_t)v + 1];
      z = xyz[3 * (size_t)best_u + 2] - xyz[3 * (size_t)v + 2];
      const float len = sqrtf(x * x + y * y + z * z);
      x = x / len; y = y / len; z = z / len;
    }
    out[3 * blockIdx.x] = x; out[3 * blockIdx.x + 1] = y; out[3 * blockIdx.x + 2] = z;
  }
}

__global__ __launch_bounds__(kBlock) void k_tb_count(tb::Args A, uint32_t T, PlanResult* __restrict__ res)
{
  const uint32_t t = blockIdx.x;
  const int lane = threadIdx.x & 63, wid = threadIdx.x >> 6;
  const TbTile W = A.tiles[t];
  for (uint32_t p = blockIdx.y * (kBlock / 64) + wid; p < A.NP; p += gridDim.y * (kBlock / 64)) {
    const float dt = A.D[tb::slot_addr(A.vaddr[A.target[p]], A.NP, p)];
    const float goal_dist = goal_cut(dt, A.offset, A.target[p]).cut;
    const float* sl = A.D + ((size_t)W.soff * A.NP + (size_t)p * W.sl);
    uint32_t c = 0;
    for (uint32_t i = lane; i < W.nv; i += 64) { const float d = sl[i]; c += (d < inf_f() && d <= goal_dist) ? 1u : 0u; }
    c = wave_sum(c);
    if (lane == 0 && c) atomicAdd(&res[p].settled, (unsigned long long)c);
  }
}

__global__ __launch_bounds__(kBlock) void k_tb_popped(tb::Args A, uint32_t p, uint32_t V, float* __restrict__ out)
{
  const float dt = A.D[tb::slot_addr(A.vaddr[A.target[p]], A.NP, p)];
  const float goal_dist = goal_cut(dt, A.offset, A.target[p]).cut;
  const uint32_t stride = gridDim.x * kBlock;
  for (uint32_t v = blockIdx.x * kBlock + threadIdx.x; v < V; v += stride) {
    const float d = A.D[tb::slot_addr(A.vaddr[v], A.NP, p)];
    out[v] = (d <= goal_dist) ? d : inf_f();
  }
}

__global__ __launch_bounds__(kBlock) void k_popped(const float* __restrict__ dist, uint32_t target, double offset, uint32_t V, float* __restrict__ out)
{
  const float dt = dist[target];
  const float goal_dist = goal_cut(dt, offset, target).cut;
  const uint32_t stride = gridDim.x * kBlock;
  for (uint32_t v = blockIdx.x * kBlock + threadIdx.x; v < V; v += stride) { const float d = dist[v]; out[v] = (d <= goal_dist) ? d : inf_f(); }
}

struct TbTables {
  bool built = false, w_valid = false;
  uint32_t ntiles = 0, max_nh = 0;
  uint64_t S = 0;
  size_t nrec = 0, nexp = 0;
  std::vector<uint32_t> vert_tile;
  DevBuf<uint32_t> d_verts;
  DevBuf<TbTile> d_tiles; DevBuf<uint32_t> d_stream, d_wsrc; DevBuf<TbExp> d_exps;
  DevBuf<uint32_t> d_vstream, d_vwsrc, d_vtile, d_vgroups; DevBuf<TbvExp> d_vexps; size_t nvrec = 0;
  DevBuf<uint2> d_vaddr; DevBuf<uint32_t> d_vert_tile;
  DevBuf<uint16_t> d_fin_src; DevBuf<uint32_t> d_fin_wsrc; DevBuf<float> d_fin_w; DevBuf<TbFinOvf> d_fin_ovf; DevBuf<uint32_t> d_fin_ovf_wsrc; DevBuf<float> d_fin_ovf_w;
  DevBuf<uint32_t> d_ghost_gid, d_fin_order; size_t fin_n = 0, fin_novf = 0; bool fin_w_valid = false; uint32_t max_sl = 0;
};

struct TbBatch {
  uint32_t cap_np = 0;
  DevBuf<float> D; DevBuf<uint32_t> pend; DevBuf<uint8_t> pflag; DevBuf<uint32_t> pairs; DevBuf<uint16_t> bucket; DevBuf<uint32_t> bcnt; DevBuf<uint2> items;
  DevBuf<tb::Ctl> ctl; PinnedBuf<tb::Ctl> h_ctl;
  DevBuf<unsigned long long> wstat; DevBuf<struct FinRec> d_recs;
  DevBuf<uint32_t> marr[2];
  DevBuf<float> thr, bnd; DevBuf<uint32_t> seed, target;
  GraphExec graph[2]; tb::Args graph_args[2]{};
  DevBuf<float> D2; bool d2_clean = false; uint32_t d2_clean_np = 0, d2_wanted_np = 0;
};

struct TbState : TbTables, TbBatch {
  uint32_t T = 120;
  int kernel = 0;
  uint32_t min_batch = 48;
  float band_mult = 2.0f;
  int iters_per_replay = 16, waves_per_cu = 0;
  Stream fill_stream; Event fill_done;
  Event warm_ev[4]; float ms_warm = 0.f, ms_warm_fin = 0.f;
  tb::Ctl last{};
  bool count_pending = false;
};

}

#ifdef MNAV_TB_TIMING
extern "C" int mnav_debug_tb_timing(unsigned long long* out)
{
  if (hipMemcpyFromSymbol(out, HIP_SYMBOL(g_tb_timing), sizeof(unsigned long long) * 8) != hipSuccess) return -1;
  unsigned long long z[8] = { 0, 0, 0, 0, 0, 0, 0, 0 };
  return hipMemcpyToSymbol(HIP_SYMBOL(g_tb_timing), z, sizeof(z)) == hipSuccess ? 0 : -1;
}
#endif
```

### mesh_navigation_amd/csrc/mnav_tb_build.h

```cpp
#pragma once
#include <algorithm>
#include <cmath>
#include <cstdint>
#include <cstring>
#include <numeric>
#include <stdexcept>
#include <vector>

#include "mnav_build.h"

namespace mnav {

struct TbExp { uint32_t u, soff, sl, off; };

struct TbTile {
  uint32_t soff;
  uint32_t sl;
  uint32_t nv;
  uint32_t nh;
  uint32_t sweep_off;
  uint32_t sweep_chunks;
  uint32_t pre_off, pre_chunks;
  uint32_t post_off, post_chunks;
  uint32_t exp_off, exp_n;
  uint32_t v0;
  uint32_t goff;
  uint32_t ovf_off, ovf_n;
};
static_assert(sizeof(TbTile) == 64, "TbTile is read as one 64-byte scalar load");

constexpr uint32_t kTbChunk = 64;
constexpr uint32_t kTbBlock = 16;
constexpr uint32_t kTbBlocksPerChunk = 4;
constexpr uint32_t kTbGhostEdges = 5;
constexpr uint32_t kTbGhostEnd = 1u << 4;
constexpr uint32_t kTbTileEnd = 1u << 6;
constexpr uint32_t kTbOrderShift = 12;
constexpr uint32_t kTbInfBits = 0x7f800000u;
constexpr uint32_t kTbDirty = 0x80000000u;

constexpr uint32_t kTbFinSlots = 8;
constexpr uint16_t kTbFinNone = 0xFFFFu;
struct TbFinOvf { uint32_t y, src, wsrc, pad; };

struct TbvExp { uint32_t rows, soff, sl, off, n, pad[3]; };
static_assert(sizeof(TbvExp) == 32, "read as two 16-byte loads");

struct HostTb {
  std::vector<uint16_t> fin_src; std::vector<uint32_t> fin_wsrc; std::vector<TbFinOvf> fin_ovf;
  std::vector<uint32_t> ghost_gid;
  uint32_t T = 0, ntiles = 0, V = 0;
  uint64_t S = 0;
  uint32_t max_nh = 0, max_sl = 0;
  std::vector<TbTile> tiles;
  std::vector<uint32_t> stream;
  std::vector<uint32_t> wsrc;
  std::vector<uint32_t> vstream, vwsrc;
  std::vector<uint32_t> vtile;
  std::vector<TbvExp> vexps;
  std::vector<uint32_t> vgroups;
  std::vector<TbExp> exps;
  std::vector<uint32_t> verts;
  std::vector<uint32_t> vert_tile, vert_local;
};

namespace detail {
inline void tb_bisect(std::vector<uint32_t>& ids, size_t lo, size_t hi, size_t k, const float* xyz, uint32_t T, std::vector<uint32_t>& cuts)
{
  const size_t n = hi - lo;
  if (k <= 1) { cuts.push_back((uint32_t)hi); return; }
  float mn[3] = { INFINITY, INFINITY, INFINITY }, mx[3] = { -INFINITY, -INFINITY, -INFINITY };
  for (size_t i = lo; i < hi; ++i)
    for (int q = 0; q < 3; ++q) { const float x = xyz[3 * (size_t)ids[i] + q]; mn[q] = std::min(mn[q], x); mx[q] = std::max(mx[q], x); }
  int ax = 0;
  for (int q = 1; q < 3; ++q) if (mx[q] - mn[q] > mx[ax] - mn[ax]) ax = q;
  auto less = [&](uint32_t a, uint32_t b) {
    const float xa = xyz[3 * (size_t)a + ax], xb = xyz[3 * (size_t)b + ax];
    return xa < xb || (xa == xb && a < b);
  };
  int ax2 = (ax + 1) % 3;
  { const int o = (ax + 2) % 3; if (mx[o] - mn[o] > mx[ax2] - mn[ax2]) ax2 = o; }
  const size_t kl = k / 2, kr = k - kl;
  const size_t target = (size_t)((double)n * (double)kl / (double)k);
  const size_t f_lo = std::max<size_t>(n > kr * (size_t)T ? n - kr * (size_t)T : 1, 1), f_hi = std::min(kl * (size_t)T, n - 1);
  const size_t w = (size_t)(2.0 * std::sqrt((double)n)) + 8;
  const size_t a = target > w ? target - w : 0, b = std::min(target + w, n - 1);
  if (a > 0) std::nth_element(ids.begin() + lo, ids.begin() + lo + a, ids.begin() + hi, less);
  if (b + 1 < n) std::nth_element(ids.begin() + lo + a, ids.begin() + lo + b, ids.begin() + hi, less);
  std::sort(ids.begin() + lo + a, ids.begin() + lo + b + 1, less);
  auto gap_at = [&](size_t c) { return xyz[3 * (size_t)ids[lo + c] + ax] - xyz[3 * (size_t)ids[lo + c - 1] + ax]; };
  float maxgap = 0.f;
  for (size_t c = a + 1; c <= b; ++c) maxgap = std::max(maxgap, gap_at(c));
  const size_t c_lo = std::min(std::max(f_lo, a + 1), b), c_hi = std::max(std::min(f_hi, b), c_lo);
  size_t cut = std::min(std::max(target, c_lo), c_hi); float best = -1.f;
  for (size_t c = c_lo; c <= c_hi; ++c) {
    const float gap = gap_at(c);
    const size_t dc = c > target ? c - target : target - c, db = cut > target ? cut - target : target - cut;
    if (gap > best * 1.0001f + 1e-12f || (gap >= best && dc < db)) { best = gap; cut = c; }
  }
  if (best < 0.5f * maxgap) {
    cut = std::min(std::max(target, c_lo), c_hi);
    size_t rl = a, rr = b + 1;
    for (size_t c = cut; c > a; --c) if (gap_at(c) >= 0.5f * maxgap) { rl = c; break; }
    for (size_t c = cut + 1; c <= b; ++c) if (gap_at(c) >= 0.5f * maxgap) { rr = c; break; }
    std::sort(ids.begin() + lo + rl, ids.begin() + lo + rr, [&](uint32_t p, uint32_t q) {
      const float xp = xyz[3 * (size_t)p + ax2], xq = xyz[3 * (size_t)q + ax2];
      return xp < xq || (xp == xq && p < q);
    });
  }
  tb_bisect(ids, lo, lo + cut, kl, xyz, T, cuts);
  tb_bisect(ids, lo + cut, hi, kr, xyz, T, cuts);
}
}

inline void tb_div_magic(uint32_t d, uint32_t* magic, uint32_t* shift)
{
  if (d <= 1u) { *magic = 0u; *shift = 0u; return; }
  uint32_t s = 31u - (uint32_t)__builtin_clz(d);
  if ((d & (d - 1u)) == 0u) s -= 1u;
  *magic = (uint32_t)(((1ull << (32u + s)) + d - 1ull) / d); *shift = s;
}
inline uint32_t tb_div_by_magic(uint32_t n, uint32_t d, uint32_t magic, uint32_t shift)
{
  return d <= 1u ? n : ((uint32_t)(((uint64_t)n * magic) >> 32) >> shift);
}

inline uint32_t tb_sweep_index(uint32_t j, uint32_t q) { return 4u * q + j; }

constexpr uint32_t kTbvSources = 6;
constexpr uint32_t kTbvGhostRows = 64;
constexpr uint32_t kTbvSrc = 0x2000u, kTbvDst = 0xA000u;
constexpr uint32_t kTbvTileWords = 12;
constexpr uint32_t kTbvGhostEnd = 1u, kTbvTileEnd = 2u;
inline void tbv_set_source(uint32_t* blk, uint32_t k, uint32_t row)
{
  static const uint32_t dw[6] = { 0, 1, 1, 2, 2, 3 }, sh[6] = { 16, 0, 16, 0, 16, 0 };
  blk[dw[k]] = (blk[dw[k]] & ~(0xFFFFu << sh[k])) | ((kTbvSrc | row) << sh[k]);
}
inline void tbv_init_block(uint32_t* blk, uint32_t row, uint32_t mode = kTbvDst)
{
  for (uint32_t q = 0; q < kTbBlock; ++q) blk[q] = 0u;
  blk[0] = mode | row;
  for (uint32_t k = 0; k < kTbvSources; ++k) { tbv_set_source(blk, k, row); blk[8 + k] = 0x7f800000u; }
}
inline uint32_t tbv_target(const uint32_t* blk) { return blk[0] & 0xFFu; }
inline uint32_t tbv_flags(const uint32_t* blk) { return blk[3] >> 16; }
inline uint32_t tbv_source(const uint32_t* blk, uint32_t k)
{
  static const uint32_t dw[6] = { 0, 1, 1, 2, 2, 3 }, sh[6] = { 16, 0, 16, 0, 16, 0 };
  return (blk[dw[k]] >> sh[k]) & 0xFFu;
}
inline uint32_t tbv_append(std::vector<uint32_t>& stream, std::vector<uint32_t>& wsrc, std::vector<uint32_t>& blocks, std::vector<uint32_t>& bw,
                           uint32_t pad_row, uint32_t pad_mode, uint32_t min_chunks, uint32_t* chunks)
{
  const uint32_t first = (uint32_t)(stream.size() / kTbChunk);
  uint32_t n = (uint32_t)((blocks.size() / kTbBlock + kTbBlocksPerChunk - 1) / kTbBlocksPerChunk);
  n = std::max(n, min_chunks);
  while (blocks.size() < (size_t)n * kTbChunk) { const size_t at = blocks.size(); blocks.resize(at + kTbBlock); bw.resize(at + kTbBlock, 0xFFFFFFFFu); tbv_init_block(&blocks[at], pad_row, pad_mode); }
  for (uint32_t c = 0; c < n; ++c) {
    const size_t at = stream.size();
    stream.resize(at + kTbChunk); wsrc.resize(at + kTbChunk);
    for (uint32_t j = 0; j < kTbBlocksPerChunk; ++j)
      for (uint32_t q = 0; q < kTbBlock; ++q) {
        stream[at + tb_sweep_index(j, q)] = blocks[(size_t)c * kTbChunk + kTbBlock * j + q];
        wsrc[at + tb_sweep_index(j, q)] = bw[(size_t)c * kTbChunk + kTbBlock * j + q];
      }
  }
  *chunks = n;
  return first;
}

inline HostTb build_tb(const HostTopology& t, const float* xyz, uint32_t T)
{
  if (T == 0 || T > 255 || (T & 3)) throw std::invalid_argument("tile-batch engine: T must be a multiple of 4 below 256");
  HostTb H;
  const uint32_t V = t.V;
  H.T = T; H.V = V;
  H.verts.resize(V);
  std::iota(H.verts.begin(), H.verts.end(), 0u);
  std::vector<uint32_t> cuts;
  if (V) detail::tb_bisect(H.verts, 0, V, std::max<size_t>(1, (size_t)std::ceil((double)V / (0.9 * T))), xyz, T, cuts);
  H.ntiles = (uint32_t)cuts.size();
  H.vert_tile.assign(V, 0); H.vert_local.assign(V, 0);
  H.tiles.assign(H.ntiles, TbTile{});
  {
    uint32_t b = 0;
    for (uint32_t tl = 0; tl < H.ntiles; ++tl) {
      std::sort(H.verts.begin() + b, H.verts.begin() + cuts[tl]);
      H.tiles[tl].v0 = b; H.tiles[tl].nv = cuts[tl] - b;
      for (uint32_t i = b; i < cuts[tl]; ++i) { H.vert_tile[H.verts[i]] = tl; H.vert_local[H.verts[i]] = i - b; }
      b = cuts[tl];
    }
  }
  std::vector<std::vector<uint32_t>> ghosts(H.ntiles);
  auto gkey = [&](uint32_t v) { return ((uint64_t)H.vert_tile[v] << 32) | H.vert_local[v]; };
  for (uint32_t tl = 0; tl < H.ntiles; ++tl) {
    auto& g = ghosts[tl];
    const TbTile& L = H.tiles[tl];
    for (uint32_t i = 0; i < L.nv; ++i) {
      const uint32_t v = H.verts[L.v0 + i];
      for (uint32_t k = t.row_ptr[v]; k < t.row_ptr[v + 1]; ++k) if (H.vert_tile[t.nbr_u[k]] != tl) g.push_back(t.nbr_u[k]);
    }
    std::sort(g.begin(), g.end(), [&](uint32_t a, uint32_t b) { return gkey(a) < gkey(b); });
    g.erase(std::unique(g.begin(), g.end()), g.end());
    TbTile& W = H.tiles[tl];
    W.nh = (uint32_t)g.size();
    W.sl = T + ((W.nh + 3u) & ~3u);
    W.soff = (uint32_t)H.S;
    if (H.S + W.sl > 0xFFFFFFFFull) throw std::invalid_argument("tile-batch engine: mesh too large for 32-bit slice offsets");
    H.S += W.sl;
    H.max_nh = std::max(H.max_nh, W.nh); H.max_sl = std::max(H.max_sl, W.sl);
  }
  auto ghost_slot = [&](uint32_t tl, uint32_t v) -> uint32_t {
    const auto& g = ghosts[tl];
    const auto it = std::lower_bound(g.begin(), g.end(), v, [&](uint32_t a, uint32_t b) { return gkey(a) < gkey(b); });
    return (uint32_t)(it - g.begin());
  };
  H.fin_src.assign((size_t)H.ntiles * kTbFinSlots * T, kTbFinNone);
  H.fin_wsrc.assign((size_t)H.ntiles * kTbFinSlots * T, kNone);
  for (uint32_t tl = 0; tl < H.ntiles; ++tl) {
    TbTile& W = H.tiles[tl];
    W.goff = (uint32_t)H.ghost_gid.size();
    H.ghost_gid.insert(H.ghost_gid.end(), ghosts[tl].begin(), ghosts[tl].end());
    W.ovf_off = (uint32_t)H.fin_ovf.size();
    for (uint32_t y = 0; y < W.nv; ++y) {
      const uint32_t v = H.verts[W.v0 + y];
      uint32_t n = 0;
      for (uint32_t k = t.row_ptr[v]; k < t.row_ptr[v + 1]; ++k, ++n) {
        const uint32_t u = t.nbr_u[k];
        const uint32_t si = (H.vert_tile[u] == tl) ? H.vert_local[u] : T + ghost_slot(tl, u);
        if (si >= kTbFinNone) throw std::invalid_argument("tile-batch engine: a slice is too long for the finalize tables");
        if (n < kTbFinSlots) { const size_t at = ((size_t)tl * kTbFinSlots + n) * T + y; H.fin_src[at] = (uint16_t)si; H.fin_wsrc[at] = k; }
        else H.fin_ovf.push_back(TbFinOvf{ y, si, k, 0u });
      }
    }
    W.ovf_n = (uint32_t)H.fin_ovf.size() - W.ovf_off;
  }
  const uint32_t kRow = 256;
  uint32_t in_chunk = 0;
  uint32_t last_target = kNone;
  auto open_block = [&]() -> size_t {
    if (in_chunk == kTbBlocksPerChunk) { in_chunk = 0; last_target = kNone; }
    const size_t at = H.stream.size();
    H.stream.resize(at + kTbBlock, 0u); H.wsrc.resize(at + kTbBlock, kNone);
    ++in_chunk;
    return at;
  };
  auto chunk_prev = [&]() -> uint32_t { return (in_chunk == 0 || in_chunk == kTbBlocksPerChunk) ? kNone : last_target; };
  auto init_sweep_block = [&](size_t at, uint32_t row, uint32_t prev) {
    for (int q = 0; q <= 7; ++q) H.stream[at + q] = row * kRow;
    if (prev != kNone) H.stream[at + 1] = prev * kRow;
    for (int q = 8; q <= 14; ++q) H.stream[at + q] = kTbInfBits;
  };
  auto noop_sweep_block = [&]() {
    const uint32_t row = (last_target == 0u) ? 1u : 0u;
    const uint32_t prev = chunk_prev();
    const size_t at = open_block();
    init_sweep_block(at, row, prev);
    last_target = row;
  };
  auto close_chunk = [&](bool sweep) {
    if (in_chunk == 0) return;
    while (in_chunk < kTbBlocksPerChunk) { if (sweep) noop_sweep_block(); else open_block(); }
    in_chunk = 0; last_target = kNone;
  };
  std::vector<uint16_t> order;
  std::vector<std::pair<uint32_t, uint32_t>> srcs;
  std::vector<uint32_t> ts;
  for (uint32_t tl = 0; tl < H.ntiles; ++tl) {
    TbTile& W = H.tiles[tl];
    const auto& g = ghosts[tl];
    float mn[3] = { INFINITY, INFINITY, INFINITY }, mx[3] = { -INFINITY, -INFINITY, -INFINITY };
    for (uint32_t i = 0; i < W.nv; ++i)
      for (int k = 0; k < 3; ++k) { const float x = xyz[3 * (size_t)H.verts[W.v0 + i] + k]; mn[k] = std::min(mn[k], x); mx[k] = std::max(mx[k], x); }
    int a0 = 0, a1 = 1;
    {
      int idx[3] = { 0, 1, 2 };
      std::sort(idx, idx + 3, [&](int x, int y) { return (mx[x] - mn[x]) > (mx[y] - mn[y]) || ((mx[x] - mn[x]) == (mx[y] - mn[y]) && x < y); });
      a0 = std::min(idx[0], idx[1]); a1 = std::max(idx[0], idx[1]);
    }
    W.sweep_off = (uint32_t)(H.stream.size() / kTbChunk);
    static const float dirs[4][2] = { { 1, 1 }, { -1, 1 }, { -1, -1 }, { 1, -1 } };
    uint32_t order_chunks[4] = { 0, 0, 0, 0 };
    std::vector<uint32_t> vs[4], vw[4];
    for (int o = 0; o < 4; ++o) {
      order.resize(W.nv);
      for (uint32_t i = 0; i < W.nv; ++i) order[i] = (uint16_t)i;
      std::stable_sort(order.begin(), order.end(), [&](uint16_t x, uint16_t y) {
        const float* px = &xyz[3 * (size_t)H.verts[W.v0 + x]]; const float* py = &xyz[3 * (size_t)H.verts[W.v0 + y]];
        return dirs[o][0] * px[a0] + dirs[o][1] * px[a1] < dirs[o][0] * py[a0] + dirs[o][1] * py[a1];
      });
      for (uint32_t i = 0; i < W.nv; ++i) {
        const uint32_t y = order[i], v = H.verts[W.v0 + y];
        uint32_t k6 = kTbvSources; size_t at = 0;
        for (uint32_t k = t.row_ptr[v]; k < t.row_ptr[v + 1]; ++k) {
          if (H.vert_tile[t.nbr_u[k]] != tl) continue;
          if (k6 == kTbvSources) { at = vs[o].size(); vs[o].resize(at + kTbBlock); vw[o].resize(at + kTbBlock, kNone); tbv_init_block(&vs[o][at], kTbvGhostRows + y); k6 = 0; }
          tbv_set_source(&vs[o][at], k6, kTbvGhostRows + H.vert_local[t.nbr_u[k]]); vw[o][at + 8 + k6] = k; ++k6;
        }
      }
      const size_t first = H.stream.size() / kTbChunk;
      for (uint32_t i = 0; i < W.nv; ++i) {
        const uint32_t y = order[i], v = H.verts[W.v0 + y];
        srcs.clear();
        for (uint32_t k = t.row_ptr[v]; k < t.row_ptr[v + 1]; ++k)
          if (H.vert_tile[t.nbr_u[k]] == tl) srcs.push_back({ H.vert_local[t.nbr_u[k]], k });
        while (!srcs.empty()) {
          if (chunk_prev() == y) noop_sweep_block();
          const uint32_t prev = chunk_prev();
          const size_t at = open_block();
          init_sweep_block(at, y, prev);
          last_target = y;
          uint32_t slot = 1;
          if (prev != kNone) {
            for (size_t e = 0; e < srcs.size(); ++e)
              if (srcs[e].first == prev) { H.wsrc[at + 8] = srcs[e].second; srcs.erase(srcs.begin() + e); break; }
            slot = 2;
          }
          while (slot <= 7 && !srcs.empty()) {
            H.stream[at + slot] = srcs.front().first * kRow; H.wsrc[at + 7 + slot] = srcs.front().second;
            srcs.erase(srcs.begin()); ++slot;
          }
        }
      }
      close_chunk(true);
      order_chunks[o] = (uint32_t)(H.stream.size() / kTbChunk - first);
    }
    W.sweep_chunks = std::max(std::max(order_chunks[0], order_chunks[1]), std::max(order_chunks[2], order_chunks[3]));
    {
      std::vector<uint32_t> st2, ws2;
      size_t src = (size_t)W.sweep_off * kTbChunk;
      for (int o = 0; o < 4; ++o) {
        const size_t len = (size_t)order_chunks[o] * kTbChunk;
        st2.insert(st2.end(), H.stream.begin() + src, H.stream.begin() + src + len);
        ws2.insert(ws2.end(), H.wsrc.begin() + src, H.wsrc.begin() + src + len);
        src += len;
        for (uint32_t c = order_chunks[o]; c < W.sweep_chunks; ++c)
          for (uint32_t j = 0; j < kTbBlocksPerChunk; ++j) {
            const size_t at = st2.size();
            st2.resize(at + kTbBlock, 0u); ws2.resize(at + kTbBlock, kNone);
            for (int q = 0; q <= 7; ++q) st2[at + q] = (j & 1u) * kRow;
            if (j) st2[at + 1] = ((j - 1u) & 1u) * kRow;
            for (int q = 8; q <= 14; ++q) st2[at + q] = kTbInfBits;
          }
      }
      H.stream.resize((size_t)W.sweep_off * kTbChunk); H.wsrc.resize((size_t)W.sweep_off * kTbChunk);
      H.stream.insert(H.stream.end(), st2.begin(), st2.end()); H.wsrc.insert(H.wsrc.end(), ws2.begin(), ws2.end());
    }
    for (size_t c = (size_t)W.sweep_off; c < (size_t)W.sweep_off + 4u * W.sweep_chunks; ++c)
      for (uint32_t j = 1; j < kTbBlocksPerChunk; ++j) {
        const uint32_t* K = &H.stream[c * kTbChunk + kTbBlock * j];
        const uint32_t* Ws = &H.wsrc[c * kTbChunk + kTbBlock * j];
        const uint32_t prev = K[-(int)kTbBlock];
        bool ok = K[0] != prev && K[1] == prev;
        for (int q = 2; q <= 7; ++q) ok = ok && !(K[q] == prev && Ws[7 + q] != kNone);
        if (!ok) throw std::logic_error("tile-batch streams: a follower block breaks the forwarding rules");
      }
    for (size_t c = (size_t)W.sweep_off; c < (size_t)W.sweep_off + 4u * W.sweep_chunks; ++c) {
      uint32_t tmp[kTbChunk], tmpw[kTbChunk];
      std::copy(H.stream.begin() + c * kTbChunk, H.stream.begin() + (c + 1) * kTbChunk, tmp);
      std::copy(H.wsrc.begin() + c * kTbChunk, H.wsrc.begin() + (c + 1) * kTbChunk, tmpw);
      for (uint32_t j = 0; j < kTbBlocksPerChunk; ++j)
        for (uint32_t q = 0; q < kTbBlock; ++q) {
          H.stream[c * kTbChunk + tb_sweep_index(j, q)] = tmp[kTbBlock * j + q];
          H.wsrc[c * kTbChunk + tb_sweep_index(j, q)] = tmpw[kTbBlock * j + q];
        }
    }
    uint32_t v_sweep_off = 0, v_sweep_chunks = 0;
    {
      size_t vblocks = 0;
      for (int o = 0; o < 4; ++o) vblocks = std::max(vblocks, vs[o].size() / kTbBlock);
      const uint32_t vchunks = (uint32_t)((vblocks + kTbBlocksPerChunk - 1) / kTbBlocksPerChunk);
      for (int o = 0; o < 4; ++o) {
        uint32_t n = 0;
        const uint32_t first = tbv_append(H.vstream, H.vwsrc, vs[o], vw[o], kTbvGhostRows, kTbvDst, vchunks, &n);
        if (o == 0) { v_sweep_off = first; v_sweep_chunks = n; }
      }
    }
    float cen[2] = { 0.f, 0.f };
    for (uint32_t i = 0; i < W.nv; ++i) { const float* q = &xyz[3 * (size_t)H.verts[W.v0 + i]]; cen[0] += q[a0]; cen[1] += q[a1]; }
    if (W.nv) { cen[0] /= (float)W.nv; cen[1] /= (float)W.nv; }
    auto ghost_order = [&](uint32_t gv) -> uint32_t {
      const float d0 = cen[0] - xyz[3 * (size_t)gv + a0], d1 = cen[1] - xyz[3 * (size_t)gv + a1];
      uint32_t best = 0; float bv = -INFINITY;
      for (uint32_t o = 0; o < 4; ++o) { const float sc = dirs[o][0] * d0 + dirs[o][1] * d1; if (sc > bv) { bv = sc; best = o; } }
      return best;
    };
    auto emit_ghost_stream = [&](bool post) {
      const size_t first = H.stream.size() / kTbChunk;
      std::vector<size_t> chunk_at;
// ... 121 lines not shown
```

### mesh_navigation_amd/csrc/mnav_tb_finalize.h

```cpp
#pragma once

namespace {

typedef float f32x3_u __attribute__((ext_vector_type(3), aligned(4)));

struct FinRec { float* dist; uint32_t* pred; float* vm; uint32_t seed; float cut; uint32_t tie; uint32_t pad_[3]; };
static_assert(sizeof(FinRec) == 48, "FinRec: 12 dwords");
constexpr uint32_t kFinRecWords = 12;

struct FinTb {
  const uint16_t* src; const float* w; const TbFinOvf* ovf; const float* ovf_w;
  const uint32_t* verts; const uint32_t* ghost_gid; const uint32_t* order;
  const float* xyz; float* const* vecmaps;
  const Plan* plans; PlanResult* res; uint32_t* mismatch; const FinRec* recs;
  uint32_t plans_per_wave, tiles_per_xcd, max_sl;
};

__global__ __launch_bounds__(kBlock) void k_tb_fin_plans(tb::Args A, const Plan* __restrict__ plans, float* const* __restrict__ vecmaps, FinRec* __restrict__ recs)
{
  const uint32_t p = blockIdx.x * kBlock + threadIdx.x;
  if (p >= A.NP) return;
  const Plan& P = plans[p];
  const float dt = A.D[tb::slot_addr(A.vaddr[A.target[p]], A.NP, p)];
  const GoalCut gc = goal_cut(dt, A.offset, A.target[p]);
  Ctl r; memset(&r, 0, sizeof(r));
  r.armed = dt < inf_f() ? 1u : 0u; r.goal_dist = gc.goal; r.thr = inf_f(); r.thr_fixed = inf_f();
  r.it = (int32_t)A.ctl->iters; r.done = 1u; r.overflow = (A.ctl->err || A.ctl->n_cand[0]) ? 1u : 0u;
  P.ctl[0] = r; P.ctl[1] = r;
  FinRec fr; memset(&fr, 0, sizeof(fr));
  fr.dist = P.dist; fr.pred = P.pred; fr.vm = vecmaps ? vecmaps[p] : nullptr; fr.seed = A.seed[p]; fr.cut = gc.cut; fr.tie = gc.tie;
  recs[p] = fr;
}

__global__ __launch_bounds__(kBlock) void k_tb_fin_weights(size_t n, const uint32_t* __restrict__ wsrc, const Nbr* __restrict__ nbr, float* __restrict__ w)
{
  const size_t stride = (size_t)gridDim.x * kBlock;
  for (size_t i = (size_t)blockIdx.x * kBlock + threadIdx.x; i < n; i += stride) w[i] = (wsrc[i] == kNone) ? inf_f() : nbr[wsrc[i]].w;
}

#ifndef MNAV_FIN_WAVES
#define MNAV_FIN_WAVES 4
#endif
#ifndef MNAV_FIN_OCC
#define MNAV_FIN_OCC 3
#endif
constexpr int kFinWaves = MNAV_FIN_WAVES;
#ifndef MNAV_FIN_NOTAB
constexpr uint32_t kFinTabSlots = 6;
#else
constexpr uint32_t kFinTabSlots = 0;
#endif
constexpr uint32_t kFinTabRows = 128, kFinTabWords = 3 * kFinTabSlots * kFinTabRows, kFinNoSlot = 255;
__host__ __device__ constexpr uint32_t fin_lds_words(uint32_t max_sl, bool vecmap) { return 5u * max_sl + (vecmap ? kFinTabWords : 0u); }
template <int T>
__global__ __launch_bounds__(64 * kFinWaves, MNAV_FIN_OCC) void k_tb_finalize(tb::Args A, FinTb F)
{
  extern __shared__ __attribute__((aligned(16))) uint32_t fin_lds_all[];
  const int lane = threadIdx.x & 63, wave = threadIdx.x >> 6;
  uint32_t* const fin_lds = fin_lds_all + (size_t)wave * fin_lds_words(F.max_sl, F.vecmaps != nullptr);
  float* const ltab = reinterpret_cast<float*>(fin_lds + 5u * F.max_sl);
  const uint32_t xcd = blockIdx.x & 7u, j = blockIdx.x >> 3;
  const uint32_t grp = xcd * F.tiles_per_xcd + j % F.tiles_per_xcd, pg = j / F.tiles_per_xcd;
  const uint32_t t_raw = grp * kFinWaves + wave;
  const bool live = t_raw < A.ntiles;
#ifdef MNAV_FIN_BISECTION_ORDER
  const uint32_t t = live ? t_raw : A.ntiles - 1u;
#else
  const uint32_t t = F.order[live ? t_raw : A.ntiles - 1u];
#endif
  const uint32_t p_beg = pg * F.plans_per_wave, p_end = min(p_beg + F.plans_per_wave, A.NP);
  if (grp * kFinWaves >= A.ntiles || p_beg >= p_end) return;
  const TbTile W = A.tiles[t];
  uint32_t* const ld = fin_lds;
  uint32_t* const lgid = fin_lds + F.max_sl;
  float* const lxyz = reinterpret_cast<float*>(fin_lds + 2 * F.max_sl);
  const uint32_t NP = A.NP;
  for (uint32_t i = lane; i < W.sl; i += 64) {
    uint32_t g = kNone;
    if (i < W.nv) g = F.verts[W.v0 + i];
    else if (i >= (uint32_t)T && i - T < W.nh) g = F.ghost_gid[W.goff + (i - T)];
    lgid[i] = g;
    if (F.vecmaps && g != kNone) { lxyz[3 * i] = F.xyz[3 * (size_t)g]; lxyz[3 * i + 1] = F.xyz[3 * (size_t)g + 1]; lxyz[3 * i + 2] = F.xyz[3 * (size_t)g + 2]; }
  }
  uint32_t ys[2] = { (uint32_t)lane, (uint32_t)lane + 64u };
  bool own[2]; uint32_t gid[2];
  uint32_t src[2][kTbFinSlots], srck[2][kTbFinSlots]; float wt[2][kTbFinSlots];
#pragma unroll
  for (int v = 0; v < 2; ++v) {
    own[v] = live && ys[v] < W.nv;
#pragma unroll
    for (int k = 0; k < (int)kTbFinSlots; ++k) {
      const size_t at = ((size_t)t * kTbFinSlots + k) * T + (own[v] ? ys[v] : 0u);
      src[v][k] = own[v] ? (uint32_t)F.src[at] : (uint32_t)kTbFinNone;
      wt[v][k] = own[v] ? F.w[at] : inf_f();
    }
  }
  __builtin_amdgcn_wave_barrier();
#pragma unroll
  for (int v = 0; v < 2; ++v) {
    gid[v] = own[v] ? lgid[ys[v]] : kNone;
#ifdef MNAV_FIN_TILEMAJOR_EXPERIMENT
    if (own[v]) gid[v] = min(t * (uint32_t)T + ys[v], 999999u);
#endif
#pragma unroll
    for (int k = 0; k < (int)kTbFinSlots; ++k)
      if (src[v][k] == kTbFinNone) src[v][k] = ys[v] < (uint32_t)T ? ys[v] : 0u;
#pragma unroll
    for (int k = 0; k < (int)kTbFinSlots; ++k) srck[v][k] = src[v][k] | ((uint32_t)k << 16);
  }
  float px[2] = { 0.f, 0.f }, py[2] = { 0.f, 0.f }, pz[2] = { 0.f, 0.f };
  if (F.vecmaps) {
#pragma unroll
    for (int v = 0; v < 2; ++v) if (own[v]) { px[v] = lxyz[3 * ys[v]]; py[v] = lxyz[3 * ys[v] + 1]; pz[v] = lxyz[3 * ys[v] + 2]; }
#pragma unroll
    for (int v = 0; v < 2; ++v) if (own[v]) {
#pragma unroll
      for (int k = 0; k < (int)kFinTabSlots; ++k) {
        const uint32_t sx = src[v][k];
        float x = lxyz[3 * sx] - px[v], y = lxyz[3 * sx + 1] - py[v], z = lxyz[3 * sx + 2] - pz[v];
        const float len = sqrtf(x * x + y * y + z * z);
        x = x / len; y = y / len; z = z / len;
        float* const tp = ltab + (uint32_t)k * kFinTabRows + ys[v];
        tp[0] = x; tp[kFinTabSlots * kFinTabRows] = y; tp[2 * kFinTabSlots * kFinTabRows] = z;
      }
    }
  }
  MNAV_GLOBAL const float* const gD = as_global(A.D) + (size_t)W.soff * NP;
  const uint32_t i0 = lane, i1 = lane + 64u, i2 = lane + 128u, i3 = lane + 192u;
  const uint32_t slm = W.sl - 1u, j0 = min(i0, slm), j1 = min(i1, slm), j2 = min(i2, slm), j3 = min(i3, slm);
  MNAV_GLOBAL const uint32_t* const g_recs = (MNAV_GLOBAL const uint32_t*)as_global(F.recs) + min((uint32_t)lane, kFinRecWords - 1u);
  auto load_slice = [&](uint32_t p, uint32_t& rec, uint32_t (&r)[4]) {
    MNAV_GLOBAL const uint32_t* s = (MNAV_GLOBAL const uint32_t*)(gD + (size_t)p * W.sl);
    rec = g_recs[(size_t)p * kFinRecWords];
    r[0] = s[j0]; r[1] = s[j1]; r[2] = s[j2]; r[3] = s[j3];
  };
  uint32_t cur[4], nxt[4], rcur, rnxt;
  load_slice(p_beg, rcur, cur);
  rnxt = rcur;
  uint32_t bad = 0;
  for (uint32_t p = p_beg; p < p_end; ++p) {
#ifndef MNAV_FIN_NOSYNC
    __syncthreads();
#endif
    if (p + 1 < p_end) load_slice(p + 1, rnxt, nxt);
    auto rw = [&](int k) { return (uint32_t)__builtin_amdgcn_readlane((int)rcur, k); };
    MNAV_GLOBAL float* const g_dist = (MNAV_GLOBAL float*)(uintptr_t)(((unsigned long long)rw(1) << 32) | rw(0));
    MNAV_GLOBAL uint32_t* const g_pred = (MNAV_GLOBAL uint32_t*)(uintptr_t)(((unsigned long long)rw(3) << 32) | rw(2));
    MNAV_GLOBAL float* const g_vm = (MNAV_GLOBAL float*)(uintptr_t)(((unsigned long long)rw(5) << 32) | rw(4));
    const uint32_t seed = rw(6);
    const bool reached = __ballot(cur[0] != kTbInfBits || cur[1] != kTbInfBits || cur[2] != kTbInfBits || cur[3] != kTbInfBits) != 0ull;
    uint32_t cnt = 0;
    if (!reached) {
#pragma unroll
      for (int v = 0; v < 2; ++v) if (own[v]) {
        g_dist[gid[v]] = inf_f(); g_pred[gid[v]] = gid[v];
        if (g_vm) { const f32x3_u z3 = { 0.f, 0.f, 0.f }; *(MNAV_GLOBAL f32x3_u*)(g_vm + 3 * (size_t)gid[v]) = z3; }
      }
    } else {
      GoalCut gcut; gcut.goal = 0.f; gcut.cut = u2f(rw(7)); gcut.tie = rw(8);
      __builtin_amdgcn_wave_barrier();
      if (i0 < W.sl) ld[i0] = cur[0];
      if (i1 < W.sl) ld[i1] = cur[1];
      if (i2 < W.sl) ld[i2] = cur[2];
      if (i3 < W.sl) ld[i3] = cur[3];
      for (uint32_t i = lane + 256u; i < W.sl; i += 64) ld[i] = ((MNAV_GLOBAL const uint32_t*)(gD + (size_t)p * W.sl))[i];
      __builtin_amdgcn_wave_barrier();
#pragma unroll
      for (int v = 0; v < 2; ++v) {
        const uint32_t dyb = ld[ys[v]];
        const float dy = u2f(dyb);
        uint32_t sum[kTbFinSlots], dsb[kTbFinSlots];
        bool at_cut = false;
#pragma unroll
        for (int k = 0; k < (int)kTbFinSlots; ++k) {
          dsb[k] = ld[src[v][k]];
          const float ds = u2f(dsb[k]);
          at_cut |= ds == gcut.cut;
          sum[k] = (ds < gcut.cut) ? f2u(ds + wt[v][k]) : kTbInfBits;
        }
        const uint32_t m = min(min(min(sum[0], sum[1]), min(sum[2], sum[3])), min(min(sum[4], sum[5]), min(sum[6], sum[7])));
        const bool is_seed = gid[v] == seed;
        const bool cut = dy > gcut.cut;
        uint32_t val = cut ? m : dyb;
        uint32_t c[kTbFinSlots];
#pragma unroll
        for (int k = 0; k < (int)kTbFinSlots; ++k) c[k] = (sum[k] == val) ? dsb[k] : kTbInfBits;
        const uint32_t bd = min(min(min(c[0], c[1]), min(c[2], c[3])), min(min(c[4], c[5]), min(c[6], c[7])));
        uint32_t best = ys[v] | (kFinNoSlot << 16), nbest = 0;
#pragma unroll
        for (int k = (int)kTbFinSlots - 1; k >= 0; --k) { const bool hit = c[k] == bd; best = hit ? srck[v][k] : best; nbest += hit ? 1u : 0u; }
        uint32_t best_s = best & 0xFFFFu, bk = best >> 16;
        const bool finite = val != kTbInfBits;
        unsigned long long key = finite && bd != kTbInfBits ? (((unsigned long long)bd << 32) | lgid[best_s]) : ~0ull;
        uint32_t nbad = (m < val && !is_seed) ? 1u : 0u;
        if (own[v] && (at_cut || (finite && nbest > 1u) || W.ovf_n)) {
          nbad = 0u;
#pragma unroll
          for (int k = 0; k < (int)kTbFinSlots; ++k) {
            const float ds = u2f(dsb[k]);
            bool ex = ds < inf_f() && ds < gcut.cut;
            if (ds == gcut.cut && ds < inf_f()) ex = lgid[src[v][k]] < gcut.tie;
            sum[k] = ex ? f2u(ds + wt[v][k]) : kTbInfBits;
          }
          val = cut ? kTbInfBits : dyb;
          if (cut) {
#pragma unroll
            for (int k = 0; k < (int)kTbFinSlots; ++k) val = min(val, sum[k]);
          }
          key = ~0ull; best_s = ys[v]; bk = kFinNoSlot;
#pragma unroll
          for (int k = 0; k < (int)kTbFinSlots; ++k) {
            if (sum[k] < val && !is_seed) ++nbad;
            if (sum[k] == val && val != kTbInfBits) {
              const unsigned long long kk = ((unsigned long long)dsb[k] << 32) | lgid[src[v][k]];
              if (kk < key) { key = kk; best_s = src[v][k]; }
            }
          }
          for (uint32_t e = 0; e < W.ovf_n; ++e) {
            const TbFinOvf o = F.ovf[W.ovf_off + e];
            if (o.y != ys[v]) continue;
            const uint32_t db = ld[o.src], g2 = lgid[o.src];
            if (!expanded_source(gcut, u2f(db), g2)) continue;
            const uint32_t sm = f2u(u2f(db) + F.ovf_w[W.ovf_off + e]);
            if (cut && sm < val) { val = sm; key = ~0ull; }
            else if (sm < val && !is_seed) ++nbad;
            if (sm == val && val != kTbInfBits) {
              const unsigned long long kk = ((unsigned long long)db << 32) | g2;
              if (kk < key) { key = kk; best_s = o.src; }
            }
          }
        }
        if (!own[v]) continue;
        bad += nbad;
        uint32_t pv = gid[v];
        float outd = u2f(val);
        if (is_seed) { outd = dy; ++cnt; }
        else {
          if (val != kTbInfBits && key == ~0ull) ++bad;
          if (val != kTbInfBits) { pv = (uint32_t)key; ++cnt; }
        }
#ifdef MNAV_FIN_NOSTORE
        if (MNAV_FIN_NOSTORE == 1) { bad += (f2u(outd) ^ pv) == 0x12345u ? 1u : 0u; }
        else { g_dist[gid[v]] = outd; g_pred[gid[v]] = pv; }
#else
        g_dist[gid[v]] = outd; g_pred[gid[v]] = pv;
#endif
        if (g_vm) {
          float x = 0.f, y = 0.f, z = 0.f;
          if (pv != gid[v]) {
            if (bk < kFinTabSlots) {
              const float* const tp = ltab + bk * kFinTabRows + ys[v];
              x = tp[0]; y = tp[kFinTabSlots * kFinTabRows]; z = tp[2 * kFinTabSlots * kFinTabRows];
            } else {
              x = lxyz[3 * best_s] - px[v]; y = lxyz[3 * best_s + 1] - py[v]; z = lxyz[3 * best_s + 2] - pz[v];
              const float len = sqrtf(x * x + y * y + z * z);
              x = x / len; y = y / len; z = z / len;
            }
          }
          const f32x3_u o3 = { x, y, z };
#ifdef MNAV_FIN_NOSTORE
          bad += (f2u(x) ^ f2u(y) ^ f2u(z)) == 0x12345u ? 1u : 0u;
#else
          *(MNAV_GLOBAL f32x3_u*)(g_vm + 3 * (size_t)gid[v]) = o3;
#endif
        }
      }
    }
    cnt = wave_sum(cnt);
    if (lane == 0 && cnt && live) atomicAdd(&F.res[p].settled, (unsigned long long)cnt);
#pragma unroll
    for (int q = 0; q < 4; ++q) cur[q] = nxt[q];
    rcur = rnxt;
  }
  bad = wave_sum(bad);
  if (lane == 0 && bad) atomicAdd(F.mismatch, bad);
}

}
```

### mesh_navigation_amd/csrc/mnav_tb_host.h

```cpp
#pragma once

void tb_free_batch(mnav_ctx* ctx)
{
  TbState& S = ctx->tb;
  if (S.fill_stream) (void)hipStreamSynchronize(S.fill_stream);
  static_cast<TbBatch&>(S) = TbBatch{};
  S.count_pending = false; ctx->tb_args_valid = false;
}

void tb_free(mnav_ctx* ctx)
{
  tb_free_batch(ctx);
  static_cast<TbTables&>(ctx->tb) = TbTables{};
}

int tb_build(mnav_ctx* ctx)
{
  TbState& S = ctx->tb;
  if (S.built) return 0;
  if (opt_set(ctx->opt.tb_tile)) S.T = opt_u32(ctx->opt.tb_tile, S.T);
  if (S.T != 64 && S.T != 96 && S.T != 120 && S.T != 128) S.T = 120;
  HostTopology t;
  t.V = ctx->V; t.E = ctx->E; t.F = ctx->F;
  t.row_ptr = ctx->h_row_ptr; t.nbr_u = ctx->h_nbr_u;
  HostTb H;
  try { H = build_tb(t, ctx->h_xyz.data(), S.T); }
  catch (const std::exception& ex) { ctx->err = ex.what(); return -1; }
  std::vector<uint2> vaddr(ctx->V);
  for (uint32_t v = 0; v < ctx->V; ++v) {
    const TbTile& W = H.tiles[H.vert_tile[v]];
    if (W.sl >= (1u << 24)) { ctx->err = "tile-batch engine: a tile has too many ghosts"; return -1; }
    vaddr[v] = make_uint2(W.soff, (W.sl << 8) | H.vert_local[v]);
  }
  HIPCHK(S.d_tiles.upload(ctx->stream, H.tiles.data(), H.tiles.size()));
  HIPCHK(S.d_stream.upload(ctx->stream, H.stream.data(), H.stream.size()));
  HIPCHK(S.d_wsrc.upload(ctx->stream, H.wsrc.data(), H.wsrc.size()));
  HIPCHK(S.d_exps.upload(ctx->stream, H.exps.data(), H.exps.size()));
  HIPCHK(S.d_vstream.upload(ctx->stream, H.vstream.data(), H.vstream.size()));
  HIPCHK(S.d_vwsrc.upload(ctx->stream, H.vwsrc.data(), H.vwsrc.size()));
  HIPCHK(S.d_vtile.upload(ctx->stream, H.vtile.data(), H.vtile.size()));
  if (H.vgroups.empty()) H.vgroups.push_back(0u);
  HIPCHK(S.d_vgroups.upload(ctx->stream, H.vgroups.data(), H.vgroups.size()));
  HIPCHK(S.d_vexps.upload(ctx->stream, H.vexps.data(), H.vexps.size()));
  HIPCHK(S.d_vaddr.upload(ctx->stream, vaddr.data(), vaddr.size()));
  HIPCHK(S.d_vert_tile.upload(ctx->stream, H.vert_tile.data(), H.vert_tile.size()));
  HIPCHK(S.d_verts.upload(ctx->stream, H.verts.data(), H.verts.size()));
  HIPCHK(S.d_fin_src.upload(ctx->stream, H.fin_src.data(), H.fin_src.size()));
  HIPCHK(S.d_fin_wsrc.upload(ctx->stream, H.fin_wsrc.data(), H.fin_wsrc.size()));
  HIPCHK(S.d_fin_ovf.upload(ctx->stream, H.fin_ovf.data(), H.fin_ovf.size()));
  {
    std::vector<uint32_t> ow(H.fin_ovf.size());
    for (size_t i = 0; i < ow.size(); ++i) ow[i] = H.fin_ovf[i].wsrc;
    HIPCHK(S.d_fin_ovf_wsrc.upload(ctx->stream, ow.data(), ow.size()));
  }
  HIPCHK(S.d_ghost_gid.upload(ctx->stream, H.ghost_gid.data(), H.ghost_gid.size()));
  {
    std::vector<uint32_t> order(H.tiles.size()), key(H.tiles.size(), 0xFFFFFFFFu);
    for (size_t t = 0; t < H.tiles.size(); ++t) {
      order[t] = (uint32_t)t;
      for (uint32_t i = 0; i < H.tiles[t].nv; ++i) key[t] = std::min(key[t], H.verts[H.tiles[t].v0 + i]);
    }
    std::stable_sort(order.begin(), order.end(), [&](uint32_t a, uint32_t b) { return key[a] < key[b]; });
    if (order.empty()) order.push_back(0u);
    HIPCHK(S.d_fin_order.upload(ctx->stream, order.data(), order.size()));
  }
  S.d_fin_w.reset(); S.d_fin_ovf_w.reset();
  S.fin_n = H.fin_src.size(); S.fin_novf = H.fin_ovf.size(); S.fin_w_valid = false; S.max_sl = H.max_sl;
  HIPCHK(S.d_fin_w.alloc(4 * std::max<size_t>(S.fin_n, 1)));
  HIPCHK(S.d_fin_ovf_w.alloc(4 * std::max<size_t>(S.fin_novf, 1)));
  HIPCHK(hipStreamSynchronize(ctx->stream));
  S.nvrec = H.vstream.size();
  S.ntiles = H.ntiles; S.S = H.S; S.nrec = H.stream.size(); S.nexp = H.exps.size(); S.max_nh = H.max_nh;
  S.vert_tile = std::move(H.vert_tile);
  S.built = true; S.w_valid = false;
  if (opt_on(ctx->opt.verbose))
    fprintf(stderr, "[mnav] tile-batch engine: T %u, %u tiles, %.2f slots per vertex, max ghosts %u, %.1f MB of streams + %.1f MB of sweep streams in the V layout\n", S.T, S.ntiles,
            ctx->V ? (double)S.S / ctx->V : 0.0, S.max_nh, (4.0 * S.nrec + 16.0 * S.nexp) / 1e6, 4.0 * S.nvrec / 1e6);
  return 0;
}

int tb_weights(mnav_ctx* ctx)
{
  TbState& S = ctx->tb;
  if (S.w_valid) return 0;
  hipLaunchKernelGGL(k_tb_weights, dim3(4096), dim3(kBlock), 0, ctx->stream, S.nrec, S.d_wsrc, ctx->d_nbr, S.d_stream);
  hipLaunchKernelGGL(k_tb_weights, dim3(4096), dim3(kBlock), 0, ctx->stream, S.nvrec, S.d_vwsrc, ctx->d_nbr, S.d_vstream);
  HIPCHK(hipGetLastError());
  S.w_valid = true; S.fin_w_valid = false;
  return 0;
}

int tb_fin_weights(mnav_ctx* ctx)
{
  TbState& S = ctx->tb;
  if (S.fin_w_valid) return 0;
  hipLaunchKernelGGL(k_tb_fin_weights, dim3(4096), dim3(kBlock), 0, ctx->stream, S.fin_n, S.d_fin_wsrc, ctx->d_nbr, S.d_fin_w);
  if (S.fin_novf) hipLaunchKernelGGL(k_tb_fin_weights, dim3(64), dim3(kBlock), 0, ctx->stream, S.fin_novf, S.d_fin_ovf_wsrc, ctx->d_nbr, S.d_fin_ovf_w);
  HIPCHK(hipGetLastError());
  S.fin_w_valid = true;
  return 0;
}

int tb_ensure_batch(mnav_ctx* ctx, uint32_t np)
{
  TbState& S = ctx->tb;
  if (np <= S.cap_np) return 0;
  tb_free_batch(ctx);
  const size_t nt = S.ntiles ? S.ntiles : 1, pairs = nt * (size_t)np;
  HIPCHK(S.D.alloc(4 * (size_t)S.S * np + 64));
  if (8 * (size_t)S.S * np <= ((size_t)96 << 30) && !opt_on(ctx->opt.tb_no_prefill)) {
    if (S.D2.alloc(4 * (size_t)S.S * np + 64) != hipSuccess) (void)hipGetLastError();
    if (S.D2 && !S.fill_stream) { HIPCHK(hipStreamCreateWithFlags(S.fill_stream.out(), hipStreamNonBlocking)); HIPCHK(hipEventCreateWithFlags(S.fill_done.out(), hipEventDisableTiming)); }
  }
  HIPCHK(S.pend.alloc(4 * pairs + 64));
  HIPCHK(S.pflag.alloc(nt * (((size_t)np + 63) / 64) + 64));
  HIPCHK(S.pairs.alloc(4 * (nt * (((size_t)np + 63) / 64) + 64)));
  HIPCHK(S.bucket.alloc(2 * pairs + 64));
  HIPCHK(S.bcnt.alloc(4 * nt));
  HIPCHK(S.items.alloc(8 * (nt + pairs / kTbItemPlans + 64)));
  HIPCHK(S.ctl.alloc(sizeof(tb::Ctl)));
  HIPCHK(S.wstat.alloc(32 * (size_t)kTbStatSlots));
  HIPCHK(S.h_ctl.alloc(sizeof(tb::Ctl)));
  for (int k = 0; k < 2; ++k) HIPCHK(S.marr[k].alloc(4 * (size_t)np));
  HIPCHK(S.thr.alloc(4 * (size_t)np)); HIPCHK(S.bnd.alloc(4 * (size_t)np));
  HIPCHK(S.seed.alloc(4 * (size_t)np)); HIPCHK(S.target.alloc(4 * (size_t)np));
  HIPCHK(S.d_recs.alloc(sizeof(FinRec) * (size_t)np));
  S.cap_np = np;
  return 0;
}

int tb_fill(mnav_ctx* ctx, void* p, size_t bytes, uint32_t v)
{
  const size_t n16 = (bytes + 15) / 16;
  uint32_t g = (uint32_t)std::min<size_t>((n16 + kBlock - 1) / kBlock, 256 * 32);
  if (g < 1) g = 1;
  hipLaunchKernelGGL(k_tb_fill, dim3(g), dim3(kBlock), 0, ctx->stream, (u32x4*)p, n16, v);
  HIPCHK(hipGetLastError());
  return 0;
}

int tb_launch_iterations(mnav_ctx* ctx, const tb::Args& A, int count, uint32_t waves)
{
  const uint32_t gp = (A.NP + kBlock - 1) / kBlock;
  for (int j = 0; j < count; ++j) {
    const int par = j & 1;
    hipLaunchKernelGGL(k_tb_plan, dim3(gp), dim3(kBlock), 0, ctx->stream, A, par);
    hipLaunchKernelGGL(k_tb_pairs, dim3((A.n_flag16 + kBlock * kTbPairUnits - 1) / (kBlock * kTbPairUnits)), dim3(kBlock), 0, ctx->stream, A);
    hipLaunchKernelGGL(k_tb_scan, dim3(kTbScanWaves / (kBlock / 64)), dim3(kBlock), 0, ctx->stream, A, par);
    hipLaunchKernelGGL(k_tb_items, dim3((A.ntiles + kBlock - 1) / kBlock), dim3(kBlock), 0, ctx->stream, A);
    if (ctx->tb.kernel == 1) hipLaunchKernelGGL((k_tbv_solve<120>), dim3(waves), dim3(64), 0, ctx->stream, A, ctx->tb.d_vtile, ctx->tb.d_vstream, ctx->tb.d_vgroups, ctx->tb.d_vexps, par);
    else if (ctx->tb.T == 64) hipLaunchKernelGGL((k_tb_solve_q<64>), dim3(waves), dim3(64), 0, ctx->stream, A, par);
    else if (ctx->tb.T == 96) hipLaunchKernelGGL((k_tb_solve_q<96>), dim3(waves), dim3(64), 0, ctx->stream, A, par);
    else if (ctx->tb.T == 120) hipLaunchKernelGGL((k_tb_solve_q<120>), dim3(waves), dim3(64), 0, ctx->stream, A, par);
    else hipLaunchKernelGGL((k_tb_solve_q<128>), dim3(waves), dim3(64), 0, ctx->stream, A, par);
  }
  hipLaunchKernelGGL(k_tb_stats, dim3(1), dim3(1024), 0, ctx->stream, A);
  HIPCHK(hipGetLastError());
  return 0;
}

int tb_fields(mnav_ctx* ctx, uint32_t n, const std::vector<PlanIn>& in, double offset, const tb::Args& A)
{
  TbState& S = ctx->tb;
  if (ensure_slots(ctx, n, false, false, ctx->want_vec)) return -1;
  if (tb_fin_weights(ctx)) return -1;
  std::vector<Plan> hp(n);
  std::vector<float*> vecs(n);
  for (uint32_t i = 0; i < n; ++i) {
    Slot& s = ctx->slots[i];
    Plan& P = hp[i];
    memset(&P, 0, sizeof(P));
    P.planner = kPlannerDijkstra; P.V = ctx->V;
    P.row_ptr = ctx->d_row_ptr.get(); P.nbr = ctx->d_nbr.get(); P.crn_ptr = ctx->d_crn_ptr.get(); P.crn = ctx->d_crn.get(); P.blocked = ctx->d_blocked.get();
    P.dist = s.dist.get(); P.pred = s.pred.get(); P.cap = ctx->V; P.ctl = s.ctl; P.cnt = s.cnt.get();
    P.offset = offset; P.max_steps = ctx->max_steps;
    for (int k = 0; k < 3; ++k) { P.seed[k] = in[i].seed[k]; P.target[k] = in[i].target[k]; P.seed_d[k] = 0.f; P.seed_expands[k] = 1; P.target_expands[k] = 1; }
    P.seed_face = kNone;
    vecs[i] = s.vecmap;
  }
  HIPCHK(hipMemcpyAsync(ctx->d_plans, hp.data(), sizeof(Plan) * n, hipMemcpyHostToDevice, ctx->stream));
  HIPCHK(hipMemcpyAsync(ctx->d_vecptrs, vecs.data(), sizeof(float*) * n, hipMemcpyHostToDevice, ctx->stream));
  HIPCHK(hipStreamSynchronize(ctx->stream));
  FinTb F{};
  F.src = S.d_fin_src; F.w = S.d_fin_w; F.ovf = S.d_fin_ovf; F.ovf_w = S.d_fin_ovf_w; F.verts = S.d_verts; F.ghost_gid = S.d_ghost_gid; F.order = S.d_fin_order;
  F.xyz = ctx->d_xyz; F.vecmaps = ctx->want_vec ? ctx->d_vecptrs : nullptr;
  F.plans = ctx->d_plans; F.res = ctx->d_res; F.mismatch = ctx->d_mismatch; F.recs = S.d_recs;
  const uint32_t groups = (S.ntiles + kFinWaves - 1u) / kFinWaves;
#ifndef MNAV_FIN_PPW
#define MNAV_FIN_PPW 64u
#endif
  F.plans_per_wave = MNAV_FIN_PPW; F.tiles_per_xcd = (groups + 7u) / 8u; F.max_sl = S.max_sl;
  hipLaunchKernelGGL(k_tb_fin_plans, dim3((n + kBlock - 1) / kBlock), dim3(kBlock), 0, ctx->stream, A, ctx->d_plans, F.vecmaps, S.d_recs);
  const uint32_t npg = (n + F.plans_per_wave - 1u) / F.plans_per_wave;
  const size_t lds = 4 * (size_t)fin_lds_words(S.max_sl, F.vecmaps != nullptr) * kFinWaves;
  const dim3 grid(8u * F.tiles_per_xcd * npg);
  if (S.T == 64) hipLaunchKernelGGL((k_tb_finalize<64>), grid, dim3(64 * kFinWaves), lds, ctx->stream, A, F);
  else if (S.T == 96) hipLaunchKernelGGL((k_tb_finalize<96>), grid, dim3(64 * kFinWaves), lds, ctx->stream, A, F);
  else if (S.T == 120) hipLaunchKernelGGL((k_tb_finalize<120>), grid, dim3(64 * kFinWaves), lds, ctx->stream, A, F);
  else hipLaunchKernelGGL((k_tb_finalize<128>), grid, dim3(64 * kFinWaves), lds, ctx->stream, A, F);
  HIPCHK(hipGetLastError());
  return 0;
}

int tb_clean_other(mnav_ctx* ctx)
{
  TbState& S = ctx->tb;
  if (!S.D2 || !S.fill_stream || S.d2_wanted_np == 0u || S.d2_clean) return 0;
  const uint32_t n = S.d2_wanted_np;
  S.d2_wanted_np = 0u;
  const size_t n16 = (4 * (size_t)S.S * n + 15) / 16;
  const uint32_t g = (uint32_t)std::max<size_t>(std::min<size_t>((n16 + kBlock - 1) / kBlock, 256 * 32), 1);
  hipLaunchKernelGGL(k_tb_fill, dim3(g), dim3(kBlock), 0, S.fill_stream, (u32x4*)S.D2.get(), n16, kTbInfBits);
  HIPCHK(hipEventRecord(S.fill_done, S.fill_stream));
  S.d2_clean = true; S.d2_clean_np = n;
  return 0;
}

struct TbWarmIn { const uint32_t* d_level; const float* const* d_dist; ReplanCnt* d_cnt; };

int run_dijkstra_tb(mnav_ctx* ctx, uint32_t n, const std::vector<PlanIn>& in, double offset, const TbWarmIn* warm = nullptr)
{
  TbState& S = ctx->tb;
  if (tb_build(ctx)) return -1;
  if (tb_weights(ctx)) return -1;
  if (n > 65535u) { ctx->err = "tile-batch engine: more than 65535 plans in one batch"; return -1; }
  if (tb_ensure_batch(ctx, n)) return -1;
  if (ensure_plan_tables(ctx, n)) return -1;
  if (ensure_paths(ctx, n)) return -1;
  if (!ctx->d_mismatch) HIPCHK(ctx->d_mismatch.alloc(4));
  std::vector<uint32_t> seeds(n), targets(n);
  for (uint32_t i = 0; i < n; ++i) { seeds[i] = in[i].seed[0]; targets[i] = in[i].target[0]; }
  HIPCHK(hipMemcpyAsync(S.seed, seeds.data(), 4 * (size_t)n, hipMemcpyHostToDevice, ctx->stream));
  HIPCHK(hipMemcpyAsync(S.target, targets.data(), 4 * (size_t)n, hipMemcpyHostToDevice, ctx->stream));
  HIPCHK(hipMemsetAsync(ctx->d_res, 0, sizeof(PlanResult) * n, ctx->stream));
  HIPCHK(hipMemsetAsync(ctx->d_mismatch, 0, 4, ctx->stream));
  tb::Args A{};
  A.tiles = S.d_tiles; A.stream = S.d_stream; A.exps = S.d_exps; A.D = S.D; A.pend = S.pend; A.pflag = S.pflag; A.nblk = (n + 63u) / 64u; A.NP = n; A.ntiles = S.ntiles;
  A.bucket = S.bucket; A.bcnt = S.bcnt; A.items = S.items; A.ctl = S.ctl; A.wstat = S.wstat; A.wstat_slots = kTbStatSlots;
  A.pairs = S.pairs; A.n_flag16 = (uint32_t)(((size_t)S.ntiles * A.nblk + 15u) / 16u);
  tb_div_magic(A.nblk, &A.nblk_magic, &A.nblk_shift);
  if ((size_t)S.ntiles * A.nblk >= (1ull << 31)) { ctx->err = "tile-batch engine: flag matrix beyond 2^31 entries"; return -1; }
  A.marr[0] = S.marr[0]; A.marr[1] = S.marr[1];
  A.thr = S.thr; A.bnd = S.bnd; A.seed = S.seed; A.target = S.target; A.vaddr = S.d_vaddr; A.vert_tile = S.d_vert_tile;
  A.offset = offset;
  const bool v_fits = S.T == 120 && S.max_nh <= kTbvGhostRows;
  const double density = (double)n / std::sqrt((double)std::max(S.ntiles, 1u));
  S.kernel = (v_fits && density >= 8.0) ? 1 : 0;
  if (opt_set(ctx->opt.tb_kernel)) S.kernel = (opt_u32(ctx->opt.tb_kernel, 0u) == 1u && v_fits) ? 1 : 0;
  A.item_plans = S.kernel == 1 ? 64u : kTbItemPlans;
  {
    const float band_mult = (S.kernel == 1 && density < 40.0) ? 4.0f : S.band_mult;
    float band = (ctx->delta_auto / 3.0f) * std::sqrt((float)S.T) * band_mult;
    if (opt_set(ctx->opt.tb_band_mult)) band = (ctx->delta_auto / 3.0f) * std::sqrt((float)S.T) * (float)ctx->opt.tb_band_mult;
    if (ctx->tile_band_user > 0.f) band = ctx->tile_band_user;
    A.band = band;
  }
  HIPCHK(hipEventRecord(ctx->ev[1], ctx->stream));
  if (!warm) {
    bool prefilled = false;
    if (S.D2 && S.d2_clean && S.d2_clean_np >= n) {
      std::swap(S.D, S.D2); A.D = S.D;
      HIPCHK(hipStreamWaitEvent(ctx->stream, S.fill_done, 0));
      prefilled = true;
    }
    S.d2_clean = false;
    if (!prefilled && tb_fill(ctx, S.D, 4 * (size_t)S.S * n, kTbInfBits)) return -1;
    if (tb_fill(ctx, S.pend, 4 * (size_t)S.ntiles * n, kTbInfBits)) return -1;
  }
  HIPCHK(hipMemsetAsync(S.pflag, 0, (size_t)(S.ntiles ? S.ntiles : 1) * ((n + 63u) / 64u) + 64u, ctx->stream));
  if (tb_fill(ctx, S.marr[0], 4 * (size_t)n, kTbInfBits)) return -1;
  if (tb_fill(ctx, S.marr[1], 4 * (size_t)n, kTbInfBits)) return -1;
  HIPCHK(hipMemsetAsync(S.ctl, 0, sizeof(tb::Ctl), ctx->stream));
  HIPCHK(hipMemsetAsync(S.wstat, 0, 32 * (size_t)kTbStatSlots, ctx->stream));
  HIPCHK(hipMemsetAsync(S.bcnt, 0, 4 * (size_t)(S.ntiles ? S.ntiles : 1), ctx->stream));
  if (warm) {
    if (!S.warm_ev[0]) for (auto& e : S.warm_ev) HIPCHK(hipEventCreate(e.out()));
    HIPCHK(hipMemsetAsync(warm->d_cnt, 0, sizeof(ReplanCnt) * (size_t)n, ctx->stream));
    TbWarm Wm{};
    Wm.level = warm->d_level; Wm.dist = warm->d_dist; Wm.cnt = warm->d_cnt;
    Wm.verts = S.d_verts; Wm.ghost_gid = S.d_ghost_gid; Wm.order = S.d_fin_order; Wm.T = S.T;
    const size_t groups = (size_t)std::max(S.ntiles, 1u) * ((n + 63u) / 64u);
    if (groups >= (1ull << 31)) { ctx->err = "tile-batch engine: warm start beyond 2^31 workgroups"; return -1; }
    HIPCHK(hipEventRecord(S.warm_ev[0], ctx->stream));
    if (S.ntiles) hipLaunchKernelGGL(k_tb_warm, dim3((uint32_t)groups), dim3(kWarmBlock), 0, ctx->stream, A, Wm);
    HIPCHK(hipEventRecord(S.warm_ev[1], ctx->stream));
  } else
  hipLaunchKernelGGL(k_tb_seed, dim3((n + kBlock - 1) / kBlock), dim3(kBlock), 0, ctx->stream, A);
  HIPCHK(hipGetLastError());
  HIPCHK(hipEventRecord(ctx->ev[2], ctx->stream));
  if (!warm || !S.d2_clean) S.d2_wanted_np = S.D2 ? n : 0u;

  int ncu = 256;
  (void)hipDeviceGetAttribute(&ncu, hipDeviceAttributeMultiprocessorCount, ctx->device);
  uint32_t per_cu = (uint32_t)((160u * 1024u) / (S.T * 256u + kTbQStride * 4u));
  if (S.kernel == 1) per_cu = 8u;
  if (opt_set(ctx->opt.tb_waves_per_cu)) S.waves_per_cu = (int)ctx->opt.tb_waves_per_cu;
  if (S.waves_per_cu > 0) per_cu = (uint32_t)S.waves_per_cu;
  const uint32_t waves = per_cu * (uint32_t)ncu;
  const int chunk = S.iters_per_replay & ~1;
  int gi = 0;
  for (int k = 0; k < 2; ++k) if (S.graph[k] && memcmp(&S.graph_args[k], &A, sizeof(A)) == 0) gi = k + 2;
  if (ctx->use_graph && gi < 2) {
    gi = (S.graph[0] && S.graph_args[0].D != A.D) ? 1 : 0;
    S.graph[gi].reset();
    hipGraph_t g = nullptr;
    HIPCHK(hipStreamBeginCapture(ctx->stream, hipStreamCaptureModeThreadLocal));
    const int rc = tb_launch_iterations(ctx, A, chunk, waves);
    const hipError_t e = hipStreamEndCapture(ctx->stream, &g);
    if (rc != 0 || e != hipSuccess) { ctx->err = "graph capture failed"; return -1; }
    HIPCHK(hipGraphInstantiate(S.graph[gi].out(), g, nullptr, nullptr, 0));
    (void)hipGraphDestroy(g);
    memcpy(&S.graph_args[gi], &A, sizeof(A));
  } else gi -= 2;
  int rc = 0;
  uint32_t iters = 0;
  const auto t_start = std::chrono::steady_clock::now();
  HIPCHK(hipEventRecord(ctx->evc[0], ctx->stream));
  for (;;) {
    if (std::chrono::duration<double>(std::chrono::steady_clock::now() - t_start).count() > ctx->max_wall_s) {
      ctx->err = "tile-batch iterations exceeded the wall-clock guard"; return -1;
    }
    if (ctx->use_graph) HIPCHK(hipGraphLaunch(S.graph[gi], ctx->stream));
    else if (tb_launch_iterations(ctx, A, chunk, waves)) return -1;
    iters += (uint32_t)chunk;
    HIPCHK(hipMemcpyAsync(S.h_ctl, S.ctl, sizeof(tb::Ctl), hipMemcpyDeviceToHost, ctx->stream));
    HIPCHK(hipStreamSynchronize(ctx->stream));
    if (S.h_ctl->err) { ctx->err = "tile-batch engine: sweep cap hit"; return -1; }
    if (S.h_ctl->n_cand[0] == 0u) break;
    if (ctx->cancel.load(std::memory_order_relaxed)) { rc = 1; break; }
    if (iters > ctx->max_steps) { ctx->err = "tile-batch engine: iteration cap hit"; return -1; }
  }
  HIPCHK(hipEventRecord(ctx->evc[1], ctx->stream));
  if (rc == 0 && !ctx->lazy_paths) {
    if (warm) HIPCHK(hipEventRecord(S.warm_ev[2], ctx->stream));
    if (tb_fields(ctx, n, in, offset, A)) return -1;
    if (warm) HIPCHK(hipEventRecord(S.warm_ev[3], ctx->stream));
  }
  HIPCHK(hipEventRecord(ctx->ev[3], ctx->stream));
  HIPCHK(hipEventSynchronize(ctx->evc[1]));
  ctx->ms_chunks = ev_ms(ctx->evc[0], ctx->evc[1]);
  S.last = *S.h_ctl;
  if (warm && rc == 0) {
    HIPCHK(hipEventSynchronize(S.warm_ev[3]));
    S.ms_warm = ev_ms(S.warm_ev[0], S.warm_ev[1]); S.ms_warm_fin = ev_ms(S.warm_ev[2], S.warm_ev[3]);
  }
  ctx->stats.launches = 1;
  ctx->tb_args = A; ctx->tb_args_valid = (rc == 0);
  if (opt_on(ctx->opt.trace))
    fprintf(stderr, "[mnav] tile-batch: %u iterations, %llu activations (%.1f per item), %llu items, %.2f sweeps per item, %llu wakes\n", S.h_ctl->iters,
            S.h_ctl->acts, S.h_ctl->items ? (double)S.h_ctl->acts / S.h_ctl->items : 0.0, S.h_ctl->items,
            S.h_ctl->items ? (double)S.h_ctl->sweeps / S.h_ctl->items : 0.0, S.h_ctl->wakes);
  return rc;
// ... 2 lines not shown
```

Measured before the change: 41630.

## Add wave-uniform fast finalize path and trim per-vertex slot count

```diff
diff --git a/include/mnav.h b/include/mnav.h
--- a/include/mnav.h
+++ b/include/mnav.h
@@ -249,6 +249,9 @@
 const void* mnav_device_output(const mnav_ctx* ctx, uint32_t slot, int what);
 uint64_t mnav_algorithmic_bytes(const mnav_ctx* ctx);
 int mnav_last_engine(const mnav_ctx* ctx);
+int mnav_tb_finalize_count(mnav_ctx* ctx, int on);
+int mnav_tb_finalize_classes(mnav_ctx* ctx, uint64_t out[4]);
+int mnav_tb_vertex_tiles(mnav_ctx* ctx, uint32_t* tile_out, uint32_t* ntiles_out);
 
 #ifdef __cplusplus
 }
diff --git a/mesh_navigation_amd/capi.py b/mesh_navigation_amd/capi.py
--- a/mesh_navigation_amd/capi.py
+++ b/mesh_navigation_amd/capi.py
@@ -35,6 +35,7 @@
     "mnav_fleet_paths", "mnav_fleet_walks", "mnav_fleet_stats",
     "mnav_upload_face_normals", "mnav_fleet_plans", "mnav_fleet_walk_plans",
     "mnav_set_option", "mnav_get_option", "mnav_shard_set_goal_tie", "mnav_last_engine",
+    "mnav_tb_finalize_count", "mnav_tb_finalize_classes", "mnav_tb_vertex_tiles",
 ]
 
 
@@ -298,6 +299,12 @@
     L.mnav_algorithmic_bytes.argtypes = [vp]
     L.mnav_last_engine.restype = C.c_int
     L.mnav_last_engine.argtypes = [vp]
+    L.mnav_tb_finalize_count.restype = C.c_int
+    L.mnav_tb_finalize_count.argtypes = [vp, C.c_int]
+    L.mnav_tb_finalize_classes.restype = C.c_int
+    L.mnav_tb_finalize_classes.argtypes = [vp, vp]
+    L.mnav_tb_vertex_tiles.restype = C.c_int
+    L.mnav_tb_vertex_tiles.argtypes = [vp, vp, C.POINTER(u32)]
     L.mnav_fleet_paths.restype = C.c_int
     L.mnav_fleet_paths.argtypes = [vp, u32] + [vp] * 9 + [C.c_uint64, vp]
     L.mnav_fleet_walks.restype = C.c_int
@@ -783,6 +790,23 @@
         if e in (5, 21) and self.replan_warm_stats()["live"]:
             return _warm_name(1 if e == 21 else 0)
         return _engine_name(e)
+
+    def tb_finalize_count(self, on: bool = True):
+        if self._L.mnav_tb_finalize_count(self._h, 1 if on else 0) != 0:
+            raise RuntimeError(f"mnav_tb_finalize_count: {self._err()}")
+
+    def tb_finalize_classes(self) -> dict:
+        out = np.zeros(4, np.uint64)
+        if self._L.mnav_tb_finalize_classes(self._h, _p(out)) != 0:
+            raise RuntimeError(f"mnav_tb_finalize_classes: {self._err()}")
+        return dict(unreached=int(out[0]), inside=int(out[1]), generic=int(out[2]), tie_fallback=int(out[3]))
+
+    def tb_vertex_tiles(self):
+        nt = C.c_uint32()
+        tiles = np.empty(self.V, np.uint32)
+        if self._L.mnav_tb_vertex_tiles(self._h, _p(tiles), C.byref(nt)) != 0:
+            raise RuntimeError(f"mnav_tb_vertex_tiles: {self._err()}")
+        return tiles, int(nt.value)
 
     def timing(self) -> dict:
         s = Stats()
diff --git a/mesh_navigation_amd/csrc/mnav.hip b/mesh_navigation_amd/csrc/mnav.hip
--- a/mesh_navigation_amd/csrc/mnav.hip
+++ b/mesh_navigation_amd/csrc/mnav.hip
@@ -1936,6 +1936,37 @@
   return ctx->last_engine + ((ctx->last_engine == 5 && ctx->tb.kernel == 1) ? 16 : 0);
 }
 
+int mnav_tb_finalize_count(mnav_ctx* ctx, int on)
+{
+  if (!ctx) return -1;
+  ctx->tb.fin_count = on != 0;
+  return 0;
+}
+
+int mnav_tb_finalize_classes(mnav_ctx* ctx, uint64_t out[4])
+{
+  if (!ctx || !out) return -1;
+  TbState& S = ctx->tb;
+  if (!S.fin_cls_valid || !S.d_fin_cls) { ctx->err = "mnav_tb_finalize_classes: the last batch ran no counted tile-batch finalize pass"; return -1; }
+  std::vector<unsigned long long> h(4 * (size_t)kTbStatSlots);
+  if (hipStreamSynchronize(ctx->stream) != hipSuccess || hipMemcpy(h.data(), S.d_fin_cls, 8 * h.size(), hipMemcpyDeviceToHost) != hipSuccess) {
+    ctx->err = "mnav_tb_finalize_classes: download failed"; return -1;
+  }
+  for (int k = 0; k < 4; ++k) out[k] = 0;
+  for (size_t i = 0; i < h.size(); ++i) out[i & 3u] += h[i];
+  return 0;
+}
+
+int mnav_tb_vertex_tiles(mnav_ctx* ctx, uint32_t* tile_out, uint32_t* ntiles_out)
+{
+  if (!ctx) return -1;
+  const TbState& S = ctx->tb;
+  if (!S.built || S.vert_tile.size() != ctx->V) { ctx->err = "mnav_tb_vertex_tiles: the tile-batch engine has not been built for this mesh"; return -1; }
+  if (tile_out) memcpy(tile_out, S.vert_tile.data(), 4 * (size_t)ctx->V);
+  if (ntiles_out) *ntiles_out = S.ntiles;
+  return 0;
+}
+
 #ifdef MNAV_TILE_TIMING
 int mnav_debug_tile_timing(unsigned long long* out, unsigned int cap)
 {
diff --git a/mesh_navigation_amd/csrc/mnav_options.h b/mesh_navigation_amd/csrc/mnav_options.h
--- a/mesh_navigation_amd/csrc/mnav_options.h
+++ b/mesh_navigation_amd/csrc/mnav_options.h
@@ -19,6 +19,7 @@
   X(tile_band) X(rounds_band_mult)                                                                                                       \
   X(tb_tile)                                                       \
   X(tb_no_prefill) X(tb_band_mult) X(tb_waves_per_cu)                                                                                    \
+  X(tb_fin_fast)          \
   X(tb_kernel)            \
   X(async_wg_per_cu) X(async_wg_per_plan) X(async_max_s)                                                                                 \
   X(async_band_mult)                              \
diff --git a/mesh_navigation_amd/csrc/mnav_tb.h b/mesh_navigation_amd/csrc/mnav_tb.h
--- a/mesh_navigation_amd/csrc/mnav_tb.h
+++ b/mesh_navigation_amd/csrc/mnav_tb.h
@@ -763,6 +763,8 @@
   DevBuf<uint2> d_vaddr; DevBuf<uint32_t> d_vert_tile;
   DevBuf<uint16_t> d_fin_src; DevBuf<uint32_t> d_fin_wsrc; DevBuf<float> d_fin_w; DevBuf<TbFinOvf> d_fin_ovf; DevBuf<uint32_t> d_fin_ovf_wsrc; DevBuf<float> d_fin_ovf_w;
   DevBuf<uint32_t> d_ghost_gid, d_fin_order; size_t fin_n = 0, fin_novf = 0; bool fin_w_valid = false; uint32_t max_sl = 0;
+  bool fin_high_slots = false;
+  DevBuf<unsigned long long> d_fin_cls; bool fin_cls_valid = false;
 };
 
 struct TbBatch {
@@ -786,6 +788,7 @@
   Event warm_ev[4]; float ms_warm = 0.f, ms_warm_fin = 0.f;
   tb::Ctl last{};
   bool count_pending = false;
+  bool fin_count = false;
 };
 
 }
diff --git a/mesh_navigation_amd/csrc/mnav_tb_build.h b/mesh_navigation_amd/csrc/mnav_tb_build.h
--- a/mesh_navigation_amd/csrc/mnav_tb_build.h
+++ b/mesh_navigation_amd/csrc/mnav_tb_build.h
@@ -46,7 +46,16 @@
 struct TbvExp { uint32_t rows, soff, sl, off, n, pad[3]; };
 static_assert(sizeof(TbvExp) == 32, "read as two 16-byte loads");
 
+inline bool tb_fin_high_slots(const std::vector<uint16_t>& fin_src, uint32_t ntiles, uint32_t T)
+{
+  for (uint32_t tl = 0; tl < ntiles; ++tl)
+    for (uint32_t k = 6; k < kTbFinSlots; ++k)
+      for (uint32_t y = 0; y < T; ++y) if (fin_src[((size_t)tl * kTbFinSlots + k) * T + y] != kTbFinNone) return true;
+  return false;
+}
+
 struct HostTb {
+  bool fin_high_slots = false;
   std::vector<uint16_t> fin_src; std::vector<uint32_t> fin_wsrc; std::vector<TbFinOvf> fin_ovf;
   std::vector<uint32_t> ghost_gid;
   uint32_t T = 0, ntiles = 0, V = 0;
@@ -236,6 +245,7 @@
     }
     W.ovf_n = (uint32_t)H.fin_ovf.size() - W.ovf_off;
   }
+  H.fin_high_slots = tb_fin_high_slots(H.fin_src, H.ntiles, T);
   const uint32_t kRow = 256;
   uint32_t in_chunk = 0;
   uint32_t last_target = kNone;
diff --git a/mesh_navigation_amd/csrc/mnav_tb_finalize.h b/mesh_navigation_amd/csrc/mnav_tb_finalize.h
--- a/mesh_navigation_amd/csrc/mnav_tb_finalize.h
+++ b/mesh_navigation_amd/csrc/mnav_tb_finalize.h
@@ -14,6 +14,8 @@
   const float* xyz; float* const* vecmaps;
   const Plan* plans; PlanResult* res; uint32_t* mismatch; const FinRec* recs;
   uint32_t plans_per_wave, tiles_per_xcd, max_sl;
+  uint32_t fast;
+  unsigned long long* cls;
 };
 
 __global__ __launch_bounds__(kBlock) void k_tb_fin_plans(tb::Args A, const Plan* __restrict__ plans, float* const* __restrict__ vecmaps, FinRec* __restrict__ recs)
@@ -52,9 +54,11 @@
 #endif
 constexpr uint32_t kFinTabRows = 128, kFinTabWords = 3 * kFinTabSlots * kFinTabRows, kFinNoSlot = 255;
 __host__ __device__ constexpr uint32_t fin_lds_words(uint32_t max_sl, bool vecmap) { return 5u * max_sl + (vecmap ? kFinTabWords : 0u); }
-template <int T>
+constexpr uint32_t kFinLdsTailWords = 4;
+template <int T, int NS>
 __global__ __launch_bounds__(64 * kFinWaves, MNAV_FIN_OCC) void k_tb_finalize(tb::Args A, FinTb F)
 {
+  static_assert(NS >= 2 && NS >= (int)kFinTabSlots && NS <= (int)kTbFinSlots, "slots per vertex");
   extern __shared__ __attribute__((aligned(16))) uint32_t fin_lds_all[];
   const int lane = threadIdx.x & 63, wave = threadIdx.x >> 6;
   uint32_t* const fin_lds = fin_lds_all + (size_t)wave * fin_lds_words(F.max_sl, F.vecmaps != nullptr);
@@ -75,6 +79,9 @@
   uint32_t* const lgid = fin_lds + F.max_sl;
   float* const lxyz = reinterpret_cast<float*>(fin_lds + 2 * F.max_sl);
   const uint32_t NP = A.NP;
+  volatile uint32_t* const l_max_sl = fin_lds_all + (size_t)kFinWaves * fin_lds_words(F.max_sl, F.vecmaps != nullptr);
+  if (lane == 0) *l_max_sl = F.max_sl;
+  auto gid_of = [&](uint32_t slot) -> uint32_t { return ld[slot + *l_max_sl]; };
   for (uint32_t i = lane; i < W.sl; i += 64) {
     uint32_t g = kNone;
     if (i < W.nv) g = F.verts[W.v0 + i];
@@ -84,12 +91,12 @@
   }
   uint32_t ys[2] = { (uint32_t)lane, (uint32_t)lane + 64u };
   bool own[2]; uint32_t gid[2];
-  uint32_t src[2][kTbFinSlots], srck[2][kTbFinSlots]; float wt[2][kTbFinSlots];
+  uint32_t src[2][NS], srck[2][NS]; float wt[2][NS];
 #pragma unroll
   for (int v = 0; v < 2; ++v) {
     own[v] = live && ys[v] < W.nv;
 #pragma unroll
-    for (int k = 0; k < (int)kTbFinSlots; ++k) {
+    for (int k = 0; k < NS; ++k) {
       const size_t at = ((size_t)t * kTbFinSlots + k) * T + (own[v] ? ys[v] : 0u);
       src[v][k] = own[v] ? (uint32_t)F.src[at] : (uint32_t)kTbFinNone;
       wt[v][k] = own[v] ? F.w[at] : inf_f();
@@ -103,10 +110,10 @@
     if (own[v]) gid[v] = min(t * (uint32_t)T + ys[v], 999999u);
 #endif
 #pragma unroll
-    for (int k = 0; k < (int)kTbFinSlots; ++k)
+    for (int k = 0; k < NS; ++k)
       if (src[v][k] == kTbFinNone) src[v][k] = ys[v] < (uint32_t)T ? ys[v] : 0u;
 #pragma unroll
-    for (int k = 0; k < (int)kTbFinSlots; ++k) srck[v][k] = src[v][k] | ((uint32_t)k << 16);
+    for (int k = 0; k < NS; ++k) srck[v][k] = src[v][k] | ((uint32_t)k << 16);
   }
   float px[2] = { 0.f, 0.f }, py[2] = { 0.f, 0.f }, pz[2] = { 0.f, 0.f };
   if (F.vecmaps) {
@@ -138,6 +145,30 @@
   load_slice(p_beg, rcur, cur);
   rnxt = rcur;
   uint32_t bad = 0;
+  const bool real0 = i0 < W.nv || (i0 >= (uint32_t)T && i0 - T < W.nh), real1 = i1 < W.nv || (i1 >= (uint32_t)T && i1 - T < W.nh);
+  const bool real2 = i2 < W.nv || (i2 >= (uint32_t)T && i2 - T < W.nh), real3 = i3 < W.nv || (i3 >= (uint32_t)T && i3 - T < W.nh);
+  const bool fast_ok = F.fast != 0u && W.ovf_n == 0u && W.sl <= 256u;
+  const uint32_t nv_live = live ? W.nv : 0u;
+  uint32_t n_unr = 0, n_in = 0, n_tie = 0;
+  auto store_fields = [&](int v, float outd, uint32_t pv, MNAV_GLOBAL float* g_dist, MNAV_GLOBAL uint32_t* g_pred) {
+    g_dist[gid[v]] = outd; g_pred[gid[v]] = pv;
+  };
+  auto unit_vec = [&](int v, bool has_pred, uint32_t bk, uint32_t best_s, bool in_table) -> f32x3_u {
+    float x = 0.f, y = 0.f, z = 0.f;
+    if (has_pred) {
+      if (in_table || bk < kFinTabSlots) {
+        const float* const tp = ltab + bk * kFinTabRows + ys[v];
+        x = tp[0]; y = tp[kFinTabSlots * kFinTabRows]; z = tp[2 * kFinTabSlots * kFinTabRows];
+      } else {
+        x = lxyz[3 * best_s] - lxyz[3 * ys[v]]; y = lxyz[3 * best_s + 1] - lxyz[3 * ys[v] + 1]; z = lxyz[3 * best_s + 2] - lxyz[3 * ys[v] + 2];
+        const float len = sqrtf(x * x + y * y + z * z);
+        x = x / len; y = y / len; z = z / len;
+      }
+    }
+    const f32x3_u o3 = { x, y, z };
+    return o3;
+  };
+  auto store_vec = [&](int v, const f32x3_u& o3, MNAV_GLOBAL float* g_vm) { *(MNAV_GLOBAL f32x3_u*)(g_vm + 3 * (size_t)gid[v]) = o3; };
   for (uint32_t p = p_beg; p < p_end; ++p) {
 #ifndef MNAV_FIN_NOSYNC
     __syncthreads();
@@ -148,16 +179,19 @@
     MNAV_GLOBAL uint32_t* const g_pred = (MNAV_GLOBAL uint32_t*)(uintptr_t)(((unsigned long long)rw(3) << 32) | rw(2));
     MNAV_GLOBAL float* const g_vm = (MNAV_GLOBAL float*)(uintptr_t)(((unsigned long long)rw(5) << 32) | rw(4));
     const uint32_t seed = rw(6);
-    const bool reached = __ballot(cur[0] != kTbInfBits || cur[1] != kTbInfBits || cur[2] != kTbInfBits || cur[3] != kTbInfBits) != 0ull;
+    GoalCut gcut; gcut.goal = 0.f; gcut.cut = u2f(rw(7)); gcut.tie = rw(8);
+    const bool out_l = (real0 && !(u2f(cur[0]) < gcut.cut)) || (real1 && !(u2f(cur[1]) < gcut.cut)) || (real2 && !(u2f(cur[2]) < gcut.cut)) || (real3 && !(u2f(cur[3]) < gcut.cut));
+    const bool inside = fast_ok && __ballot(out_l) == 0ull;
+    const bool reached = inside || __ballot(cur[0] != kTbInfBits || cur[1] != kTbInfBits || cur[2] != kTbInfBits || cur[3] != kTbInfBits) != 0ull;
     uint32_t cnt = 0;
     if (!reached) {
+      ++n_unr;
 #pragma unroll
       for (int v = 0; v < 2; ++v) if (own[v]) {
-        g_dist[gid[v]] = inf_f(); g_pred[gid[v]] = gid[v];
-        if (g_vm) { const f32x3_u z3 = { 0.f, 0.f, 0.f }; *(MNAV_GLOBAL f32x3_u*)(g_vm + 3 * (size_t)gid[v]) = z3; }
+        store_fields(v, inf_f(), gid[v], g_dist, g_pred);
+        if (g_vm) { const f32x3_u z3 = { 0.f, 0.f, 0.f }; store_vec(v, z3, g_vm); }
       }
     } else {
-      GoalCut gcut; gcut.goal = 0.f; gcut.cut = u2f(rw(7)); gcut.tie = rw(8);
       __builtin_amdgcn_wave_barrier();
       if (i0 < W.sl) ld[i0] = cur[0];
       if (i1 < W.sl) ld[i1] = cur[1];
@@ -165,30 +199,78 @@
       if (i3 < W.sl) ld[i3] = cur[3];
       for (uint32_t i = lane + 256u; i < W.sl; i += 64) ld[i] = ((MNAV_GLOBAL const uint32_t*)(gD + (size_t)p * W.sl))[i];
       __builtin_amdgcn_wave_barrier();
+      bool fast_done = false;
+      if (inside) {
+        uint32_t f_dy[2], f_best[2], f_bad = 0;
+        bool f_seed[2], tie_l = false;
+#pragma unroll
+        for (int v = 0; v < 2; ++v) {
+          const uint32_t dyb = ld[ys[v]];
+          uint32_t sum[NS], dsb[NS];
+#pragma unroll
+          for (int k = 0; k < NS; ++k) { dsb[k] = ld[src[v][k]]; sum[k] = f2u(u2f(dsb[k]) + wt[v][k]); }
+          uint32_t m = sum[0];
+#pragma unroll
+          for (int k = 1; k < NS; ++k) m = min(m, sum[k]);
+          uint32_t c[NS];
+#pragma unroll
+          for (int k = 0; k < NS; ++k) c[k] = (sum[k] == dyb) ? dsb[k] : kTbInfBits;
+          uint32_t bd = c[0];
+#pragma unroll
+          for (int k = 1; k < NS; ++k) bd = min(bd, c[k]);
+          uint32_t best = ys[v] | (kFinNoSlot << 16), nbest = 0;
+#pragma unroll
+          for (int k = NS - 1; k >= 0; --k) { const bool hit = c[k] == bd; best = hit ? srck[v][k] : best; nbest += hit ? 1u : 0u; }
+          f_seed[v] = gid[v] == seed;
+          if (own[v]) {
+            f_bad += (m < dyb && !f_seed[v]) ? 1u : 0u;
+            f_bad += (bd == kTbInfBits && !f_seed[v]) ? 1u : 0u;
+            tie_l |= nbest > 1u;
+          }
+          f_dy[v] = dyb; f_best[v] = best;
+        }
+        if (__ballot(tie_l) == 0ull) {
+          fast_done = true; ++n_in;
+          bad += f_bad;
+          cnt = nv_live;
+#pragma unroll
+          for (int v = 0; v < 2; ++v) if (own[v]) {
+            const uint32_t best_s = f_best[v] & 0xFFFFu, bk = f_best[v] >> 16;
+            const uint32_t pv = f_seed[v] ? gid[v] : lgid[best_s];
+            store_fields(v, u2f(f_dy[v]), pv, g_dist, g_pred);
+            if (g_vm) store_vec(v, unit_vec(v, pv != gid[v], bk, best_s, NS <= (int)kFinTabSlots), g_vm);
+          }
+        } else ++n_tie;
+      }
+      if (!fast_done) {
 #pragma unroll
       for (int v = 0; v < 2; ++v) {
         const uint32_t dyb = ld[ys[v]];
         const float dy = u2f(dyb);
-        uint32_t sum[kTbFinSlots], dsb[kTbFinSlots];
+        uint32_t sum[NS], dsb[NS];
         bool at_cut = false;
 #pragma unroll
-        for (int k = 0; k < (int)kTbFinSlots; ++k) {
+        for (int k = 0; k < NS; ++k) {
           dsb[k] = ld[src[v][k]];
           const float ds = u2f(dsb[k]);
           at_cut |= ds == gcut.cut;
           sum[k] = (ds < gcut.cut) ? f2u(ds + wt[v][k]) : kTbInfBits;
         }
-        const uint32_t m = min(min(min(sum[0], sum[1]), min(sum[2], sum[3])), min(min(sum[4], sum[5]), min(sum[6], sum[7])));
+        uint32_t m = sum[0];
+#pragma unroll
+        for (int k = 1; k < NS; ++k) m = min(m, sum[k]);
         const bool is_seed = gid[v] == seed;
         const bool cut = dy > gcut.cut;
         uint32_t val = cut ? m : dyb;
-        uint32_t c[kTbFinSlots];
-#pragma unroll
-        for (int k = 0; k < (int)kTbFinSlots; ++k) c[k] = (sum[k] == val) ? dsb[k] : kTbInfBits;
-        const uint32_t bd = min(min(min(c[0], c[1]), min(c[2], c[3])), min(min(c[4], c[5]), min(c[6], c[7])));
+        uint32_t c[NS];
+#pragma unroll
+        for (int k = 0; k < NS; ++k) c[k] = (sum[k] == val) ? dsb[k] : kTbInfBits;
+        uint32_t bd = c[0];
+#pragma unroll
+        for (int k = 1; k < NS; ++k) bd = min(bd, c[k]);
         uint32_t best = ys[v] | (kFinNoSlot << 16), nbest = 0;
 #pragma unroll
-        for (int k = (int)kTbFinSlots - 1; k >= 0; --k) { const bool hit = c[k] == bd; best = hit ? srck[v][k] : best; nbest += hit ? 1u : 0u; }
+        for (int k = NS - 1; k >= 0; --k) { const bool hit = c[k] == bd; best = hit ? srck[v][k] : best; nbest += hit ? 1u : 0u; }
         uint32_t best_s = best & 0xFFFFu, bk = best >> 16;
         const bool finite = val != kTbInfBits;
         unsigned long long key = finite && bd != kTbInfBits ? (((unsigned long long)bd << 32) | lgid[best_s]) : ~0ull;
@@ -196,23 +278,23 @@
         if (own[v] && (at_cut || (finite && nbest > 1u) || W.ovf_n)) {
           nbad = 0u;
 #pragma unroll
-          for (int k = 0; k < (int)kTbFinSlots; ++k) {
+          for (int k = 0; k < NS; ++k) {
             const float ds = u2f(dsb[k]);
             bool ex = ds < inf_f() && ds < gcut.cut;
-            if (ds == gcut.cut && ds < inf_f()) ex = lgid[src[v][k]] < gcut.tie;
+            if (ds == gcut.cut && ds < inf_f()) ex = gid_of(src[v][k]) < gcut.tie;
             sum[k] = ex ? f2u(ds + wt[v][k]) : kTbInfBits;
           }
           val = cut ? kTbInfBits : dyb;
           if (cut) {
 #pragma unroll
-            for (int k = 0; k < (int)kTbFinSlots; ++k) val = min(val, sum[k]);
+            for (int k = 0; k < NS; ++k) val = min(val, sum[k]);
           }
           key = ~0ull; best_s = ys[v]; bk = kFinNoSlot;
 #pragma unroll
-          for (int k = 0; k < (int)kTbFinSlots; ++k) {
+          for (int k = 0; k < NS; ++k) {
             if (sum[k] < val && !is_seed) ++nbad;
             if (sum[k] == val && val != kTbInfBits) {
-              const unsigned long long kk = ((unsigned long long)dsb[k] << 32) | lgid[src[v][k]];
+              const unsigned long long kk = ((unsigned long long)dsb[k] << 32) | gid_of(src[v][k]);
               if (kk < key) { key = kk; best_s = src[v][k]; }
             }
           }
@@ -241,32 +323,22 @@
         }
 #ifdef MNAV_FIN_NOSTORE
         if (MNAV_FIN_NOSTORE == 1) { bad += (f2u(outd) ^ pv) == 0x12345u ? 1u : 0u; }
-        else { g_dist[gid[v]] = outd; g_pred[gid[v]] = pv; }
+        else store_fields(v, outd, pv, g_dist, g_pred);
 #else
-        g_dist[gid[v]] = outd; g_pred[gid[v]] = pv;
+        store_fields(v, outd, pv, g_dist, g_pred);
 #endif
         if (g_vm) {
-          float x = 0.f, y = 0.f, z = 0.f;
-          if (pv != gid[v]) {
-            if (bk < kFinTabSlots) {
-              const float* const tp = ltab + bk * kFinTabRows + ys[v];
-              x = tp[0]; y = tp[kFinTabSlots * kFinTabRows]; z = tp[2 * kFinTabSlots * kFinTabRows];
-            } else {
-              x = lxyz[3 * best_s] - px[v]; y = lxyz[3 * best_s + 1] - py[v]; z = lxyz[3 * best_s + 2] - pz[v];
-              const float len = sqrtf(x * x + y * y + z * z);
-              x = x / len; y = y / len; z = z / len;
-            }
-          }
-          const f32x3_u o3 = { x, y, z };
+          const f32x3_u o3 = unit_vec(v, pv != gid[v], bk, best_s, false);
 #ifdef MNAV_FIN_NOSTORE
-          bad += (f2u(x) ^ f2u(y) ^ f2u(z)) == 0x12345u ? 1u : 0u;
+          bad += (f2u(o3.x) ^ f2u(o3.y) ^ f2u(o3.z)) == 0x12345u ? 1u : 0u;
 #else
-          *(MNAV_GLOBAL f32x3_u*)(g_vm + 3 * (size_t)gid[v]) = o3;
-#endif
-        }
+          store_vec(v, o3, g_vm);
+#endif
+        }
+      }
+      cnt = wave_sum(cnt);
       }
     }
-    cnt = wave_sum(cnt);
     if (lane == 0 && cnt && live) atomicAdd(&F.res[p].settled, (unsigned long long)cnt);
 #pragma unroll
     for (int q = 0; q < 4; ++q) cur[q] = nxt[q];
@@ -274,6 +346,14 @@
   }
   bad = wave_sum(bad);
   if (lane == 0 && bad) atomicAdd(F.mismatch, bad);
+  if (F.cls && live && lane == 0) {
+    unsigned long long* const c4 = F.cls + 4u * (size_t)(blockIdx.x % kTbStatSlots);
+    const uint32_t n_gen = (p_end - p_beg) - n_unr - n_in;
+    if (n_unr) atomicAdd(c4, (unsigned long long)n_unr);
+    if (n_in) atomicAdd(c4 + 1, (unsigned long long)n_in);
+    if (n_gen) atomicAdd(c4 + 2, (unsigned long long)n_gen);
+    if (n_tie) atomicAdd(c4 + 3, (unsigned long long)n_tie);
+  }
 }
 
 }
diff --git a/mesh_navigation_amd/csrc/mnav_tb_host.h b/mesh_navigation_amd/csrc/mnav_tb_host.h
--- a/mesh_navigation_amd/csrc/mnav_tb_host.h
+++ b/mesh_navigation_amd/csrc/mnav_tb_host.h
@@ -66,6 +66,7 @@
   }
   S.d_fin_w.reset(); S.d_fin_ovf_w.reset();
   S.fin_n = H.fin_src.size(); S.fin_novf = H.fin_ovf.size(); S.fin_w_valid = false; S.max_sl = H.max_sl;
+  S.fin_high_slots = H.fin_high_slots;
   HIPCHK(S.d_fin_w.alloc(4 * std::max<size_t>(S.fin_n, 1)));
   HIPCHK(S.d_fin_ovf_w.alloc(4 * std::max<size_t>(S.fin_novf, 1)));
   HIPCHK(hipStreamSynchronize(ctx->stream));
@@ -190,14 +191,22 @@
 #define MNAV_FIN_PPW 64u
 #endif
   F.plans_per_wave = MNAV_FIN_PPW; F.tiles_per_xcd = (groups + 7u) / 8u; F.max_sl = S.max_sl;
+  F.fast = (!opt_set(ctx->opt.tb_fin_fast) || opt_on(ctx->opt.tb_fin_fast)) ? 1u : 0u;
+  S.fin_cls_valid = false;
+  if (S.fin_count) {
+    if (!S.d_fin_cls) HIPCHK(S.d_fin_cls.alloc(32 * (size_t)kTbStatSlots));
+    HIPCHK(hipMemsetAsync(S.d_fin_cls, 0, 32 * (size_t)kTbStatSlots, ctx->stream));
+    F.cls = S.d_fin_cls; S.fin_cls_valid = true;
+  }
   hipLaunchKernelGGL(k_tb_fin_plans, dim3((n + kBlock - 1) / kBlock), dim3(kBlock), 0, ctx->stream, A, ctx->d_plans, F.vecmaps, S.d_recs);
   const uint32_t npg = (n + F.plans_per_wave - 1u) / F.plans_per_wave;
-  const size_t lds = 4 * (size_t)fin_lds_words(S.max_sl, F.vecmaps != nullptr) * kFinWaves;
+  const size_t lds = 4 * ((size_t)fin_lds_words(S.max_sl, F.vecmaps != nullptr) * kFinWaves + kFinLdsTailWords);
   const dim3 grid(8u * F.tiles_per_xcd * npg);
-  if (S.T == 64) hipLaunchKernelGGL((k_tb_finalize<64>), grid, dim3(64 * kFinWaves), lds, ctx->stream, A, F);
-  else if (S.T == 96) hipLaunchKernelGGL((k_tb_finalize<96>), grid, dim3(64 * kFinWaves), lds, ctx->stream, A, F);
-  else if (S.T == 120) hipLaunchKernelGGL((k_tb_finalize<120>), grid, dim3(64 * kFinWaves), lds, ctx->stream, A, F);
-  else hipLaunchKernelGGL((k_tb_finalize<128>), grid, dim3(64 * kFinWaves), lds, ctx->stream, A, F);
+  if (S.T == 64) hipLaunchKernelGGL((k_tb_finalize<64, 8>), grid, dim3(64 * kFinWaves), lds, ctx->stream, A, F);
+  else if (S.T == 96) hipLaunchKernelGGL((k_tb_finalize<96, 8>), grid, dim3(64 * kFinWaves), lds, ctx->stream, A, F);
+  else if (S.T == 120 && !S.fin_high_slots) hipLaunchKernelGGL((k_tb_finalize<120, 6>), grid, dim3(64 * kFinWaves), lds, ctx->stream, A, F);
+  else if (S.T == 120) hipLaunchKernelGGL((k_tb_finalize<120, 8>), grid, dim3(64 * kFinWaves), lds, ctx->stream, A, F);
+  else hipLaunchKernelGGL((k_tb_finalize<128, 8>), grid, dim3(64 * kFinWaves), lds, ctx->stream, A, F);
   HIPCHK(hipGetLastError());
   return 0;
 }
```

New measurement: 41770, median of 4. No clear change (+0.3%).
